# microsoft/UniSpeech

Hardware: AMD Instinct MI355X
Metric: audio-seconds/sec pretraining, WavLM-Base 15s@16kHz (higher is better)
Workload: dtype bf16; 1 GPU; WavLM-Base (12L, d=768) pretrain fwd+bwd+grad-reduce+fused-Adam, bf16, batch=32x15s per GPU, masked-pred loss (BASELINE.json configs[1]); global_batch=32, frames_per_utt=749, parallelism=dp1, optimizer=fused Adam, fp32 master, clip 10

## Files before the change

include/wavlm_hip.h:

```cpp
#ifndef WAVLM_HIP_H
#define WAVLM_HIP_H
#include <stddef.h>
#include <stdint.h>
#ifdef __cplusplus
extern "C" {
#endif

#define WAVLM_HIP_ABI_VERSION 30
int wavlm_abi_version(void);

typedef struct wavlm_gemm_desc {
  int32_t dtype;
  int32_t c_dtype;
  int32_t M, N, K, KB;
  int32_t transA, transB;
  int64_t lda, ldb, ldc;
  int64_t sA_kb, sB_kb;
  int32_t batch_o, batch_i;
  int64_t sA_o, sA_i, sB_o, sB_i, sC_o, sC_i;
  const void* A;
  const void* B;
  void* C;
  float alpha;
  int32_t epi;
// ... 54 lines not shown
                      void* stream);
#define WL_CONV_RELAYOUT_MAX 8
typedef struct {
  const void* W[WL_CONV_RELAYOUT_MAX];
  void* Wf[WL_CONV_RELAYOUT_MAX];
  void* Wb[WL_CONV_RELAYOUT_MAX];
  int32_t Cout[WL_CONV_RELAYOUT_MAX], Cin[WL_CONV_RELAYOUT_MAX], k[WL_CONV_RELAYOUT_MAX], s[WL_CONV_RELAYOUT_MAX];
  int32_t n_layers, dtype;
} wavlm_conv_relayout_desc;
int wavlm_conv_weights_relayout(const wavlm_conv_relayout_desc* d, void* stream);
int wavlm_conv_wgrad_scatter(const wavlm_conv_relayout_desc* d, int32_t accumulate, void* stream);
int wavlm_axpby(const void* x, int32_t x_dtype, void* y, int32_t y_dtype, int64_t n, float a, float b, void* stream);
int wavlm_scale_dev(void* y, int32_t dtype, int64_t n, const float* scalar, float extra, void* stream);
int wavlm_dropout(const void* x, void* y, int64_t n, float p, uint64_t seed, int32_t dtype, void* stream);
int wavlm_dropout_add(const void* x, const void* r, void* y, int64_t n, float p, uint64_t seed, int32_t dtype, void* stream);
int wavlm_replace_mix(const void* x, const void* q, const uint8_t* sel, void* y, int64_t rows, int32_t D, float p, uint64_t seed,
                      int32_t dtype, void* stream);
int wavlm_replace_mix_bwd(const void* g, const uint8_t* sel, void* dx, void* dq, int64_t rows, int32_t D, float p, uint64_t seed,
                          int32_t dtype, void* stream);
uint64_t wavlm_sumsq_workspace_bytes(void);
int wavlm_sumsq(const void* x, int32_t dtype, int64_t n, float scale, float* out, void* workspace, uint64_t ws_bytes,
                void* stream);

uint64_t wavlm_conv0_gn_workspace_bytes(int32_t B, int64_t T, int32_t C, int32_t stride);
int wavlm_conv0_gn_gelu_fwd(const void* wav, int32_t wav_dtype, const void* W, const void* gamma, const void* beta,
                            int32_t param_dtype, void* out, int32_t out_dtype, float* stats, int32_t B, int64_t T,
                            int32_t C, int32_t kw, int32_t stride, float eps, void* workspace, uint64_t ws_bytes,
                            void* stream);
uint64_t wavlm_conv0_gn_bwd_workspace_bytes(int32_t B, int64_t T, int32_t C, int32_t stride);
int wavlm_conv0_gn_gelu_bwd(const void* wav, int32_t wav_dtype, const void* W, const void* gamma, const void* beta,
                            int32_t param_dtype, const void* g, int32_t g_dtype, const float* stats, void* dW,
                            void* dgamma, void* dbeta, int32_t B, int64_t T, int32_t C, int32_t kw, int32_t stride,
                            float gscale, void* workspace, uint64_t ws_bytes, void* stream);

uint64_t wavlm_conv0_ln_fwd_workspace_bytes(void);
int wavlm_conv0_ln_gelu_fwd(const void* wav, int32_t wav_dtype, const void* W, const void* conv_bias, const void* gamma,
                            const void* beta, int32_t param_dtype, void* out, int32_t out_dtype, int32_t B, int64_t T,
                            int32_t C, int32_t kw, int32_t stride, float eps, void* workspace, uint64_t ws_bytes,
                            void* stream);
uint64_t wavlm_conv0_ln_bwd_workspace_bytes(int32_t B, int64_t T, int32_t C, int32_t stride);
int wavlm_conv0_ln_gelu_bwd(const void* wav, int32_t wav_dtype, const void* W, const void* conv_bias, const void* gamma,
                            const void* beta, int32_t param_dtype, const void* g, int32_t g_dtype, void* dW,
                            void* dconv_bias, void* dgamma, void* dbeta, int32_t B, int64_t T, int32_t C, int32_t kw,
                            int32_t stride, float eps, float gscale, void* workspace, uint64_t ws_bytes, void* stream);

int wavlm_relpos_gather(const void* emb, int32_t emb_dtype, const int32_t* bucket, float* tab, int32_t H, int32_t L,
                        void* stream);
int wavlm_relpos_scatter(const float* dtab, const int32_t* bucket, void* demb, int32_t emb_dtype, int32_t H, int32_t L,
                         int32_t num_buckets, void* stream);
int wavlm_gate_fwd(const void* x, const void* W, const void* bias, const void* grep_a, float* gate, float* ga, float* gb,
                   int32_t B, int32_t T, int32_t H, int32_t hd, int32_t dtype, int32_t param_dtype, void* stream);
uint64_t wavlm_gate_bwd_workspace_bytes(int32_t H, int32_t hd);
int wavlm_gate_bwd(const float* dgate, const void* x, const void* W, const void* grep_a, const float* ga,
                   const float* gb, void* dx, void* dW, void* dbias, void* dgrep_a, int32_t B, int32_t T, int32_t H,
                   int32_t hd, int32_t dtype, int32_t param_dtype, int32_t accumulate_params, void* workspace,
                   uint64_t ws_bytes, void* stream);
int wavlm_attn_softmax_fwd(const void* S, void* P, float* lse, const float* gate, const float* tab, const uint8_t* kpm,
                           int32_t B, int32_t H, int32_t T, int64_t ldS, int64_t ldP, int32_t s_dtype, int32_t p_dtype,
                           float p_drop, uint64_t seed, void* stream);
uint64_t wavlm_attn_softmax_bwd_workspace_bytes(int32_t B, int32_t H, int32_t T);
int wavlm_attn_softmax_bwd(const void* S, const void* dP, const float* lse, const float* gate, const float* tab,
                           const uint8_t* kpm, void* dS, float* dgate, float* dtab, int32_t dtab_accumulate, int32_t B,
                           int32_t H, int32_t T, int64_t ldS, int64_t ldP, int32_t s_dtype, int32_t p_dtype,
                           float p_drop, uint64_t seed, void* workspace, uint64_t ws_bytes, void* stream);

int wavlm_attn_fused_fwd(const void* qkv, void* O, float* lse, const float* gate, const float* tab, const uint8_t* kpm,
                         int32_t B, int32_t H, int32_t T, int32_t head_dim, float scale, float p_drop, uint64_t seed,
                         void* stream);
uint64_t wavlm_attn_fused_bwd_workspace_bytes(int32_t B, int32_t H, int32_t T);
int wavlm_attn_fused_bwd(const void* qkv, const void* O, const void* dO, const float* lse, const float* gate,
                         const float* tab, const uint8_t* kpm, void* dqkv, float* dgate, float* dtab, void* dbias,
                         int32_t dbias_dtype, int32_t dbias_accumulate, int32_t B, int32_t H, int32_t T, int32_t head_dim,
                         float scale, float p_drop, uint64_t seed, void* workspace, uint64_t ws_bytes, void* stream);
uint64_t wavlm_attn_fused_pstore_bytes(int32_t B, int32_t H, int32_t T);
uint64_t wavlm_attn_fused_dbits_bytes(int32_t B, int32_t H, int32_t T);
int wavlm_attn_fused_fwd_p(const void* qkv, void* O, float* lse, const float* gate, const float* tab, const uint8_t* kpm,
                           void* pstore, uint64_t pstore_bytes, int32_t B, int32_t H, int32_t T, int32_t head_dim, float scale,
                           float p_drop, uint64_t seed, void* stream);
int wavlm_attn_fused_bwd_p(const void* qkv, const void* O, const void* dO, const float* lse, const float* gate,
                           const float* tab, const uint8_t* kpm, const void* pstore, uint64_t pstore_bytes, void* dqkv,
                           float* dgate, float* dtab, void* dbias, int32_t dbias_dtype, int32_t dbias_accumulate, int32_t B,
                           int32_t H, int32_t T, int32_t head_dim, float scale, float p_drop, uint64_t seed, void* workspace,
                           uint64_t ws_bytes, void* stream);

uint64_t wavlm_posconv_weight_workspace_bytes(int32_t D, int32_t Cg, int32_t K);
int wavlm_posconv_weight_fwd(const void* v, const void* g, int32_t param_dtype, void* Wf, void* Wb, int32_t out_dtype,
                             float* norm, int32_t D, int32_t Cg, int32_t K, int32_t layout, void* workspace,
                             uint64_t ws_bytes, void* stream);
int wavlm_posconv_weight_bwd(const float* dWf, const void* v, const void* g, const float* norm, int32_t param_dtype,
                             void* dv, void* dg, int32_t D, int32_t Cg, int32_t K, int32_t nsplit, void* workspace,
                             uint64_t ws_bytes, void* stream);
int wavlm_posconv_group_major(const void* x, const void* aux, void* out, void* nat_out, int32_t B, int32_t T, int32_t D,
                              int32_t G, int32_t left_pad, int32_t Tp, int32_t dtype, int32_t aux_is_grad, void* stream);

int wavlm_posconv_direct_supported(int32_t Cg, int32_t K, int32_t T);
int wavlm_posconv_direct(const void* xg, const void* W, const void* bias, const void* res, void* out, void* aux,
                         int32_t B, int32_t G, int32_t T, int32_t Tp, int32_t Cg, int32_t K, int32_t gelu, void* stream);
int wavlm_posconv_dw_direct_splits(int32_t Cg, int32_t G);
int wavlm_posconv_dw_direct(const void* xg, const void* dug, float* part, int32_t B, int32_t G, int32_t T, int32_t Tp,
                            int32_t du_off, int32_t Cg, int32_t K, void* stream);

int wavlm_l2norm_fwd(const void* x, int32_t x_dtype, void* y, int32_t y_dtype, float* inv_norm, int64_t rows,
                     int32_t D, float eps, void* stream);
int wavlm_l2norm_bwd(const void* dy, const void* y, int32_t y_dtype, const float* inv_norm, void* dx, int32_t x_dtype,
                     int64_t rows, int32_t D, void* stream);
int wavlm_ce_rows(const float* logits, const int32_t* target, float* loss_rows, float* correct_rows, void* dlogits,
                  int32_t d_dtype, int64_t S, int32_t V, int64_t ld_logits, int64_t ld_dlogits, float weight,
                  int32_t flat_wrong, void* stream);

int wavlm_gather_dot(const void* X, const void* Y, int32_t dtype, const int32_t* idx, float* out, int64_t S, int32_t N,
                     int32_t D, float scale, const void* mask_raw, void* stream);
int wavlm_rows_wsum(const void* Y, int32_t dtype, const int32_t* src, const float* w, const int32_t* off, void* out,
                    int32_t out_dtype, int64_t rows, int32_t D, int32_t accumulate, void* stream);
uint64_t wavlm_bce_workspace_bytes(void);
int wavlm_bce_logits(const float* logits, const uint8_t* targets, float* dlogits, float* out, int64_t n, float gscale,
                     void* workspace, uint64_t ws_bytes, void* stream);
int wavlm_glu_fwd(const void* x, void* y, int64_t rows, int32_t F, int32_t dtype, int32_t gate, void* stream);
int wavlm_glu_bwd(const void* x, const void* dy, void* dx, int64_t rows, int32_t F, int32_t dtype, int32_t gate, void* stream);
int wavlm_act_fwd(const void* x, void* y, int64_t n, int32_t dtype, int32_t kind, void* stream);
int wavlm_act_bwd(const void* x, const void* dy, void* dx, int64_t n, int32_t dtype, int32_t kind, void* stream);
uint64_t wavlm_sum_workspace_bytes(void);
int wavlm_sum_f32(const float* x, int64_t n, float* out, void* workspace, uint64_t ws_bytes, void* stream);

int wavlm_adam_step(float* p, float* m, float* v, const void* grad, int32_t grad_dtype, void* p_lowp,
                    int32_t lowp_dtype, int64_t n, float lr, float beta1, float beta2, float eps, float weight_decay,
                    int64_t step, float grad_mult, const float* grad_mult_dev, const float* gnorm_sq, float max_norm,
                    void* stream);

uint64_t wavlm_mix_workspace_bytes(int32_t B, int64_t T);
int wavlm_mix_utterances(const float* src, float* dst, void* dst_lowp, int32_t B, int64_t T, const int32_t* ops,
                         int32_t n_ops, const int32_t* op_begin, const float* noise, int32_t normalize, float eps,
                         void* workspace, uint64_t ws_bytes, void* stream);

uint64_t wavlm_gumbel_vq_partial_rows(int64_t n);
int wavlm_gumbel_vq_fwd(const void* logits, int32_t dtype, const float* noise, uint64_t seed, float tau, int32_t training,
                        int64_t n, int32_t G, int32_t V, float* ysoft, int32_t* idx, float* part, int64_t ld_part,
                        void* stream);
int wavlm_vq_perplexity(const float* sums, int64_t n, int32_t G, int32_t V, float* out, float* dA, void* stream);
int wavlm_gumbel_vq_bwd(const void* logits, int32_t dtype, const float* ysoft, const float* dret, const float* dA,
                        const float* dppl, float tau, int64_t n, int32_t G, int32_t V, void* dlogits, void* stream);

typedef struct wavlm_layer_desc {
  int32_t B, T, D, H, F;
  int32_t pre_ln;
  int32_t param_dtype;
  int32_t dtab_accumulate;
  float eps1, eps2, scale;
  float p_drop, p_attn;
  int32_t attn_store_p;
  uint64_t seed_r1, seed_r2, seed_attn;
  const void *Wqkv, *bqkv, *Wo, *bo, *W1, *b1, *W2, *b2, *ln1_g, *ln1_b, *ln2_g, *ln2_b;
  const void *Wgate, *bgate, *grep_a;
  void *dWqkv, *dbqkv, *dWo, *dbo, *dW1, *db1, *dW2, *db2, *dln1_g, *dln1_b, *dln2_g, *dln2_b, *dWgate, *dbgate, *dgrep_a;
  void* db2_prev;
  const float* tab;
  const uint8_t* kpm;
  const void* x;
  const void* r_in;
  void* y;
  void* r_out;
  void* saved; uint64_t saved_bytes;
  void* workspace; uint64_t ws_bytes;
  const void* dy;
  const void* dr_out;
  void* dx;
  void* dr_in;
  float* dtab;
} wavlm_layer_desc;
uint64_t wavlm_layer_saved_bytes(const wavlm_layer_desc* d);
uint64_t wavlm_layer_fwd_workspace_bytes(const wavlm_layer_desc* d);
uint64_t wavlm_layer_bwd_workspace_bytes(const wavlm_layer_desc* d);
int wavlm_encoder_layer_fwd(const wavlm_layer_desc* d, void* stream);
int wavlm_encoder_layer_bwd(const wavlm_layer_desc* d, void* stream);

typedef void (*wavlm_grad_listener)(const void* base, uint64_t bytes, void* stream, void* user);
void wavlm_dp_set_listener(wavlm_grad_listener cb, void* user);

int wavlm_dp_unique_id(void* id128);
int wavlm_dp_init(int32_t rank, int32_t world, const void* id128, int32_t average);
int wavlm_dp_bucket_ready(void* base, uint64_t count, int32_t dtype, void* compute_stream);
int wavlm_dp_finish(void* compute_stream);
int wavlm_dp_destroy(void);

uint64_t wavlm_kmeans_centres_bytes(int32_t K, int32_t D);
int wavlm_kmeans_prepare(const float* C, int32_t K, int32_t D, void* image, uint64_t image_bytes, void* stream);
int wavlm_kmeans_assign(const void* X, int32_t x_dtype, int64_t N, int32_t D, int64_t ldx, const void* image, int32_t K,
                        int32_t* labels, float* min_dist, void* stream);
uint64_t wavlm_kmeans_accumulate_workspace_bytes(int64_t N, int32_t K, int32_t D);
int wavlm_kmeans_accumulate(const void* X, int32_t x_dtype, int64_t N, int32_t D, int64_t ldx, const int32_t* labels,
                            int32_t K, float* sums, int32_t* counts, void* workspace, uint64_t ws_bytes, void* stream);
int wavlm_kmeans_update(float* C, float* weights, const float* sums, const int32_t* counts, int32_t K, int32_t D,
                        int32_t mode, void* stream);

int wavlm_spk_mix_norm(const void* const* states, const int64_t* stride_b, const int64_t* stride_t, int32_t n_states,
                       int32_t dtype, const float* weights, const int32_t* lengths, int32_t B, int32_t T, int32_t D,
                       void* out, int32_t out_dtype, int64_t out_stride_b, int64_t out_stride_t, int32_t pad, float add,
                       float eps, void* stream);
int wavlm_spk_rowact(const void* x, int32_t x_dtype, int64_t x_stride_b, int64_t ldx, void* y, int32_t y_dtype,
                     int64_t y_stride_b, int64_t ldy, int32_t B, int32_t T, int32_t C, int32_t act, const float* scale,
                     const float* shift, const int32_t* lengths, float* mean_out, void* stream);
int wavlm_spk_res2(const void* x, int32_t x_dtype, int64_t x_stride_b, int64_t ldx, void* y, int32_t y_dtype,
                   int64_t y_stride_b, int64_t ldy, int32_t B, int32_t T, int32_t C, int32_t dilation, const float* w_image,
                   const float* bias, const float* scale, const float* shift, const int32_t* lengths, void* stream);
uint64_t wavlm_spk_se_workspace_bytes(int32_t B, int32_t C);
int wavlm_spk_se_residual(const void* x, int32_t x_dtype, int64_t x_stride_b, int64_t ldx, const float* mean, const void* w1,
                          const void* b1, const void* w2, const void* b2, int32_t w_dtype, const void* res, int32_t res_dtype,
                          int64_t res_stride_b, int64_t ld_res, void* out, int32_t out_dtype, int64_t out_stride_b,
                          int64_t ld_out, int32_t B, int32_t T, int32_t C, int32_t Cb, const int32_t* lengths,
                          void* workspace, uint64_t ws_bytes, void* stream);
int wavlm_spk_asp(const void* x, int32_t x_dtype, int64_t x_stride_b, int64_t ldx, const void* logits, int32_t l_dtype,
                  int64_t l_stride_b, int64_t ldl, int32_t B, int32_t T, int32_t C, const int32_t* lengths, const float* scale,
                  const float* shift, float* pooled_raw, void* out, int32_t out_dtype, void* stream);

int wavlm_diar_front(const void* const* states, const int64_t* stride_b, const int64_t* stride_t, int32_t n_states,
                     int32_t dtype, const float* weights, int32_t B, int32_t T, int32_t D, int32_t subsampling, int32_t T_out,
                     void* out, int32_t out_dtype, int64_t out_stride_b, int64_t out_stride_t, float add, float eps,
                     void* stream);
int wavlm_attn_plain_fwd(const void* qkv, void* O, int32_t B, int32_t H, int32_t T, int32_t head_dim, int32_t dtype,
                         float scale, void* stream);
int wavlm_diar_estimate(const void* z, int32_t z_dtype, int64_t z_stride_b, int64_t ldz, int32_t B, int32_t T, int32_t S,
                        int32_t E, float* activities, void* vectors, int32_t v_dtype, void* stream);

int wavlm_resample_supported(int32_t o, int32_t n, int32_t width);
int wavlm_resample_rows(const void* x, int32_t x_dtype, int64_t x_stride, int32_t B, int64_t L, const int32_t* lengths,
                        const float* table, const int32_t* first, int32_t o, int32_t n, int32_t width, void* y,
                        int32_t y_dtype, int64_t y_stride, void* stream);

int wavlm_mfcc_supported(int32_t W, int32_t S, int32_t P);
int64_t wavlm_mfcc_frames(int64_t len, int32_t W, int32_t S);
int wavlm_mfcc_rows(const void* x, int32_t x_dtype, int64_t x_stride, int32_t B, int64_t L, const int32_t* lengths, int32_t W,
                    int32_t S, int32_t P, const float* window, const float* twiddle, const int32_t* mel_idx, const float* mel_w,
                    int32_t n_mel_w, const float* dct, float* y, int64_t y_stride, int64_t Mmax, int32_t ncol, void* stream);

int wavlm_fbank_supported(int32_t W, int32_t S, int32_t P, int32_t M);
int64_t wavlm_fbank_frames(int64_t len, int32_t S, int32_t P);
int wavlm_fbank_rows(const void* x, int32_t x_dtype, int64_t x_stride, int32_t B, int64_t L, const int32_t* lengths, int32_t W,
                     int32_t S, int32_t P, int32_t M, const float* window, const float* twiddle, const int32_t* mel_idx,
                     const float* mel_w, int32_t n_mel_w, float* y, int64_t y_stride, int64_t Tmax, void* stream);

int wavlm_ctc_supported(int32_t C, int32_t Lmax);
uint64_t wavlm_ctc_workspace_bytes(int32_t B, int32_t T, int32_t Lmax);
int wavlm_ctc_loss(const void* logits, int32_t dtype, int64_t stride_b, int64_t stride_t, int32_t B, int32_t T, int32_t C,
                   const int32_t* targets, const int32_t* target_offsets, int32_t n_targets, int32_t Lmax,
                   const int32_t* input_lengths, int32_t blank, int32_t zero_infinity, const float* grad_out, float* nll,
                   void* dlogits, void* workspace, uint64_t ws_bytes, void* stream);
int wavlm_ctc_greedy(const void* logits, int32_t dtype, int64_t stride_b, int64_t stride_t, int32_t B, int32_t T, int32_t C,
                     const int32_t* input_lengths, int32_t blank, int32_t* tokens, int32_t* counts, void* stream);

int wavlm_ctc_score_supported(int32_t T, int32_t Lt);
uint64_t wavlm_ctc_score_workspace_bytes(int32_t B, int32_t T, int32_t Lt);
// ... 50 lines not shown
```

unispeech_amd/_lib.py:

```python
import ctypes as C
import os

_HERE = os.path.dirname(os.path.abspath(__file__))
LIB_PATH = os.environ.get("WAVLM_HIP_LIB") or os.path.join(_HERE, "lib", "libwavlm_hip.so")

_lib = None
ABI_VERSION = 30

F32, BF16, I16 = 0, 1, 2

c_i32, c_i64, c_u64, c_f32, c_vp = C.c_int32, C.c_int64, C.c_uint64, C.c_float, C.c_void_p


class ConvRelayoutDesc(C.Structure):
    _fields_ = [("W", c_vp * 8), ("Wf", c_vp * 8), ("Wb", c_vp * 8),
                ("Cout", c_i32 * 8), ("Cin", c_i32 * 8), ("k", c_i32 * 8), ("s", c_i32 * 8),
                ("n_layers", c_i32), ("dtype", c_i32)]


class GemmDesc(C.Structure):
    _fields_ = [
        ("dtype", c_i32), ("c_dtype", c_i32),
        ("M", c_i32), ("N", c_i32), ("K", c_i32), ("KB", c_i32),
        ("transA", c_i32), ("transB", c_i32),
        ("lda", c_i64), ("ldb", c_i64), ("ldc", c_i64),
        ("sA_kb", c_i64), ("sB_kb", c_i64),
        ("batch_o", c_i32), ("batch_i", c_i32),
        ("sA_o", c_i64), ("sA_i", c_i64), ("sB_o", c_i64), ("sB_i", c_i64), ("sC_o", c_i64), ("sC_i", c_i64),
        ("A", c_vp), ("B", c_vp), ("C", c_vp),
        ("alpha", c_f32), ("epi", c_i32),
        ("bias", c_vp), ("bias_dtype", c_i32), ("sBias_o", c_i64), ("sBias_i", c_i64),
        ("aux", c_vp), ("aux_dtype", c_i32), ("ld_aux", c_i64), ("sAux_o", c_i64), ("sAux_i", c_i64),
        ("res", c_vp), ("res_dtype", c_i32), ("ld_res", c_i64), ("sRes_o", c_i64), ("sRes_i", c_i64),
        ("accumulate", c_i32), ("split_k", c_i32),
        ("workspace", c_vp), ("ws_bytes", c_u64),
        ("colsum", c_vp), ("colsum_dtype", c_i32), ("colsum_accumulate", c_i32),
    ]


class WgradItem(C.Structure):
    _fields_ = [("dy", c_vp), ("x", c_vp), ("dW", c_vp), ("N", c_i32), ("K", c_i32)]


class LayerDesc(C.Structure):
    _fields_ = [
        ("B", c_i32), ("T", c_i32), ("D", c_i32), ("H", c_i32), ("F", c_i32),
        ("pre_ln", c_i32), ("param_dtype", c_i32), ("dtab_accumulate", c_i32),
        ("eps1", c_f32), ("eps2", c_f32), ("scale", c_f32), ("p_drop", c_f32), ("p_attn", c_f32),
        ("attn_store_p", c_i32),
        ("seed_r1", c_u64), ("seed_r2", c_u64), ("seed_attn", c_u64),
        ("Wqkv", c_vp), ("bqkv", c_vp), ("Wo", c_vp), ("bo", c_vp), ("W1", c_vp), ("b1", c_vp), ("W2", c_vp), ("b2", c_vp),
        ("ln1_g", c_vp), ("ln1_b", c_vp), ("ln2_g", c_vp), ("ln2_b", c_vp),
        ("Wgate", c_vp), ("bgate", c_vp), ("grep_a", c_vp),
        ("dWqkv", c_vp), ("dbqkv", c_vp), ("dWo", c_vp), ("dbo", c_vp), ("dW1", c_vp), ("db1", c_vp), ("dW2", c_vp),
        ("db2", c_vp), ("dln1_g", c_vp), ("dln1_b", c_vp), ("dln2_g", c_vp), ("dln2_b", c_vp),
        ("dWgate", c_vp), ("dbgate", c_vp), ("dgrep_a", c_vp),
        ("db2_prev", c_vp),
        ("tab", c_vp), ("kpm", c_vp),
        ("x", c_vp), ("r_in", c_vp), ("y", c_vp), ("r_out", c_vp),
        ("saved", c_vp), ("saved_bytes", c_u64), ("workspace", c_vp), ("ws_bytes", c_u64),
        ("dy", c_vp), ("dr_out", c_vp), ("dx", c_vp), ("dr_in", c_vp), ("dtab", c_vp),
    ]


GRAD_LISTENER = C.CFUNCTYPE(None, c_vp, c_u64, c_vp, c_vp)


SIGNATURES = {
    "wavlm_abi_version": (c_i32, []),
    "wavlm_gemm_workspace_bytes": (c_u64, [C.POINTER(GemmDesc)]),
    "wavlm_gemm": (c_i32, [C.POINTER(GemmDesc), c_vp]),
    "wavlm_gemm_grouped": (c_i32, [C.POINTER(GemmDesc), c_i32, c_vp]),
    "wavlm_grid_blocks": (c_i32, []),
    "wavlm_split_single": (c_i32, [c_i32, c_i32, c_i64, c_i32]),
    "wavlm_split_grouped": (c_i32, [c_i64, c_i64, c_i32, c_i32]),
    "wavlm_slabs_grouped": (c_i32, [c_i64, c_i64, c_i32, c_i32, c_i32]),
    "wavlm_wgrad_grouping": (c_i32, []),
    "wavlm_linear_wgrads_workspace_bytes": (c_u64, [C.POINTER(WgradItem), c_i32, c_i64]),
    "wavlm_linear_wgrads": (c_i32, [C.POINTER(WgradItem), c_i32, c_i64, c_i32, c_vp, c_u64, c_vp]),
    "wavlm_layernorm_fwd": (c_i32, [c_vp, c_vp, c_vp, c_vp, c_vp, c_vp, c_vp, c_vp, c_i64, c_i32, c_f32, c_i32, c_i32,
                                    c_i32, c_f32, c_u64, c_f32, c_u64, c_vp]),
    "wavlm_layernorm_bwd_workspace_bytes": (c_u64, [c_i32]),
    "wavlm_layernorm_bwd": (c_i32, [c_vp, c_vp, c_vp, c_vp, c_vp, c_vp, c_vp, c_vp, c_vp, c_vp, c_vp, c_vp, c_i64, c_i32, c_i32,
                                    c_i32, c_i32, c_f32, c_u64, c_f32, c_u64, c_f32, c_i32, c_i32, c_vp, c_u64, c_vp]),
    "wavlm_layernorm_bwd_seg": (c_i32, [c_vp, c_vp, c_vp, c_vp, c_vp, c_vp, c_vp, c_vp, c_vp, c_vp, c_vp, c_vp, c_i64, c_i32, c_i32,
                                        c_i32, c_i32, c_f32, c_u64, c_f32, c_u64, c_f32, c_i32, c_i32, c_i32, c_i32, c_vp, c_u64,
                                        c_vp]),
    "wavlm_colsum_workspace_bytes": (c_u64, [c_i32]),
    "wavlm_colsum": (c_i32, [c_vp, c_i64, c_i32, c_i64, c_i32, c_vp, c_vp, c_vp, c_i32, c_i32, c_vp, c_u64, c_vp]),
    "wavlm_select_rows": (c_i32, [c_vp, c_vp, c_vp, c_vp, c_vp, c_i64, c_i32, c_i32, c_i32, c_vp]),
    "wavlm_gather_rows": (c_i32, [c_vp, c_vp, c_vp, c_i64, c_i32, c_i32, c_vp]),
    "wavlm_conv_weights_relayout": (c_i32, [C.POINTER(ConvRelayoutDesc), c_vp]),
    "wavlm_conv_wgrad_scatter": (c_i32, [C.POINTER(ConvRelayoutDesc), c_i32, c_vp]),
    "wavlm_axpby": (c_i32, [c_vp, c_i32, c_vp, c_i32, c_i64, c_f32, c_f32, c_vp]),
    "wavlm_scale_dev": (c_i32, [c_vp, c_i32, c_i64, c_vp, c_f32, c_vp]),
    "wavlm_dropout": (c_i32, [c_vp, c_vp, c_i64, c_f32, c_u64, c_i32, c_vp]),
    "wavlm_dropout_add": (c_i32, [c_vp, c_vp, c_vp, c_i64, c_f32, c_u64, c_i32, c_vp]),
    "wavlm_replace_mix": (c_i32, [c_vp, c_vp, c_vp, c_vp, c_i64, c_i32, c_f32, c_u64, c_i32, c_vp]),
    "wavlm_replace_mix_bwd": (c_i32, [c_vp, c_vp, c_vp, c_vp, c_i64, c_i32, c_f32, c_u64, c_i32, c_vp]),
    "wavlm_sumsq_workspace_bytes": (c_u64, []),
    "wavlm_sumsq": (c_i32, [c_vp, c_i32, c_i64, c_f32, c_vp, c_vp, c_u64, c_vp]),
    "wavlm_conv0_gn_workspace_bytes": (c_u64, [c_i32, c_i64, c_i32, c_i32]),
    "wavlm_conv0_gn_gelu_fwd": (c_i32, [c_vp, c_i32, c_vp, c_vp, c_vp, c_i32, c_vp, c_i32, c_vp, c_i32, c_i64, c_i32,
                                        c_i32, c_i32, c_f32, c_vp, c_u64, c_vp]),
    "wavlm_conv0_gn_bwd_workspace_bytes": (c_u64, [c_i32, c_i64, c_i32, c_i32]),
    "wavlm_conv0_gn_gelu_bwd": (c_i32, [c_vp, c_i32, c_vp, c_vp, c_vp, c_i32, c_vp, c_i32, c_vp, c_vp, c_vp, c_vp,
                                        c_i32, c_i64, c_i32, c_i32, c_i32, c_f32, c_vp, c_u64, c_vp]),
    "wavlm_conv0_ln_fwd_workspace_bytes": (c_u64, []),
    "wavlm_conv0_ln_gelu_fwd": (c_i32, [c_vp, c_i32, c_vp, c_vp, c_vp, c_vp, c_i32, c_vp, c_i32, c_i32, c_i64, c_i32, c_i32,
                                        c_i32, c_f32, c_vp, c_u64, c_vp]),
    "wavlm_conv0_ln_bwd_workspace_bytes": (c_u64, [c_i32, c_i64, c_i32, c_i32]),
    "wavlm_conv0_ln_gelu_bwd": (c_i32, [c_vp, c_i32, c_vp, c_vp, c_vp, c_vp, c_i32, c_vp, c_i32, c_vp, c_vp, c_vp, c_vp, c_i32,
                                        c_i64, c_i32, c_i32, c_i32, c_f32, c_f32, c_vp, c_u64, c_vp]),
    "wavlm_relpos_gather": (c_i32, [c_vp, c_i32, c_vp, c_vp, c_i32, c_i32, c_vp]),
    "wavlm_relpos_scatter": (c_i32, [c_vp, c_vp, c_vp, c_i32, c_i32, c_i32, c_i32, c_vp]),
    "wavlm_gate_fwd": (c_i32, [c_vp, c_vp, c_vp, c_vp, c_vp, c_vp, c_vp, c_i32, c_i32, c_i32, c_i32, c_i32, c_i32,
                               c_vp]),
    "wavlm_gate_bwd_workspace_bytes": (c_u64, [c_i32, c_i32]),
    "wavlm_gate_bwd": (c_i32, [c_vp, c_vp, c_vp, c_vp, c_vp, c_vp, c_vp, c_vp, c_vp, c_vp, c_i32, c_i32, c_i32, c_i32,
                               c_i32, c_i32, c_i32, c_vp, c_u64, c_vp]),
    "wavlm_attn_softmax_fwd": (c_i32, [c_vp, c_vp, c_vp, c_vp, c_vp, c_vp, c_i32, c_i32, c_i32, c_i64, c_i64, c_i32,
                                       c_i32, c_f32, c_u64, c_vp]),
    "wavlm_attn_softmax_bwd_workspace_bytes": (c_u64, [c_i32, c_i32, c_i32]),
    "wavlm_attn_softmax_bwd": (c_i32, [c_vp, c_vp, c_vp, c_vp, c_vp, c_vp, c_vp, c_vp, c_vp, c_i32, c_i32, c_i32,
                                       c_i32, c_i64, c_i64, c_i32, c_i32, c_f32, c_u64, c_vp, c_u64, c_vp]),
    "wavlm_attn_fused_fwd": (c_i32, [c_vp, c_vp, c_vp, c_vp, c_vp, c_vp, c_i32, c_i32, c_i32, c_i32, c_f32, c_f32, c_u64,
                                     c_vp]),
    "wavlm_attn_fused_bwd_workspace_bytes": (c_u64, [c_i32, c_i32, c_i32]),
    "wavlm_attn_fused_bwd": (c_i32, [c_vp, c_vp, c_vp, c_vp, c_vp, c_vp, c_vp, c_vp, c_vp, c_vp, c_vp, c_i32, c_i32,
                                     c_i32, c_i32, c_i32, c_i32, c_f32, c_f32, c_u64, c_vp, c_u64, c_vp]),
    "wavlm_attn_fused_pstore_bytes": (c_u64, [c_i32, c_i32, c_i32]),
    "wavlm_attn_fused_dbits_bytes": (c_u64, [c_i32, c_i32, c_i32]),
    "wavlm_attn_fused_fwd_p": (c_i32, [c_vp, c_vp, c_vp, c_vp, c_vp, c_vp, c_vp, c_u64, c_i32, c_i32, c_i32, c_i32, c_f32, c_f32,
                                       c_u64, c_vp]),
    "wavlm_attn_fused_bwd_p": (c_i32, [c_vp, c_vp, c_vp, c_vp, c_vp, c_vp, c_vp, c_vp, c_u64, c_vp, c_vp, c_vp, c_vp, c_i32, c_i32,
                                       c_i32, c_i32, c_i32, c_i32, c_f32, c_f32, c_u64, c_vp, c_u64, c_vp]),
    "wavlm_posconv_weight_workspace_bytes": (c_u64, [c_i32, c_i32, c_i32]),
    "wavlm_posconv_weight_fwd": (c_i32, [c_vp, c_vp, c_i32, c_vp, c_vp, c_i32, c_vp, c_i32, c_i32, c_i32, c_i32, c_vp,
                                         c_u64, c_vp]),
    "wavlm_posconv_dw_direct_splits": (c_i32, [c_i32, c_i32]),
    "wavlm_posconv_dw_direct": (c_i32, [c_vp, c_vp, c_vp, c_i32, c_i32, c_i32, c_i32, c_i32, c_i32, c_i32, c_vp]),
    "wavlm_posconv_weight_bwd": (c_i32, [c_vp, c_vp, c_vp, c_vp, c_i32, c_vp, c_vp, c_i32, c_i32, c_i32, c_i32, c_vp, c_u64,
                                         c_vp]),
    "wavlm_posconv_direct_supported": (c_i32, [c_i32, c_i32, c_i32]),
    "wavlm_posconv_direct": (c_i32, [c_vp, c_vp, c_vp, c_vp, c_vp, c_vp, c_i32, c_i32, c_i32, c_i32, c_i32, c_i32, c_i32,
                                     c_vp]),
    "wavlm_posconv_group_major": (c_i32, [c_vp, c_vp, c_vp, c_vp, c_i32, c_i32, c_i32, c_i32, c_i32, c_i32, c_i32,
                                          c_i32, c_vp]),
    "wavlm_l2norm_fwd": (c_i32, [c_vp, c_i32, c_vp, c_i32, c_vp, c_i64, c_i32, c_f32, c_vp]),
    "wavlm_l2norm_bwd": (c_i32, [c_vp, c_vp, c_i32, c_vp, c_vp, c_i32, c_i64, c_i32, c_vp]),
    "wavlm_ce_rows": (c_i32, [c_vp, c_vp, c_vp, c_vp, c_vp, c_i32, c_i64, c_i32, c_i64, c_i64, c_f32, c_i32, c_vp]),
    "wavlm_gather_dot": (c_i32, [c_vp, c_vp, c_i32, c_vp, c_vp, c_i64, c_i32, c_i32, c_f32, c_vp, c_vp]),
    "wavlm_rows_wsum": (c_i32, [c_vp, c_i32, c_vp, c_vp, c_vp, c_vp, c_i32, c_i64, c_i32, c_i32, c_vp]),
    "wavlm_bce_workspace_bytes": (c_u64, []),
    "wavlm_bce_logits": (c_i32, [c_vp, c_vp, c_vp, c_vp, c_i64, c_f32, c_vp, c_u64, c_vp]),
    "wavlm_glu_fwd": (c_i32, [c_vp, c_vp, c_i64, c_i32, c_i32, c_i32, c_vp]),
    "wavlm_glu_bwd": (c_i32, [c_vp, c_vp, c_vp, c_i64, c_i32, c_i32, c_i32, c_vp]),
    "wavlm_act_fwd": (c_i32, [c_vp, c_vp, c_i64, c_i32, c_i32, c_vp]),
    "wavlm_act_bwd": (c_i32, [c_vp, c_vp, c_vp, c_i64, c_i32, c_i32, c_vp]),
    "wavlm_sum_workspace_bytes": (c_u64, []),
    "wavlm_sum_f32": (c_i32, [c_vp, c_i64, c_vp, c_vp, c_u64, c_vp]),
    "wavlm_adam_step": (c_i32, [c_vp, c_vp, c_vp, c_vp, c_i32, c_vp, c_i32, c_i64, c_f32, c_f32, c_f32, c_f32, c_f32,
                                c_i64, c_f32, c_vp, c_vp, c_f32, c_vp]),
    "wavlm_mix_workspace_bytes": (c_u64, [c_i32, c_i64]),
    "wavlm_mix_utterances": (c_i32, [c_vp, c_vp, c_vp, c_i32, c_i64, c_vp, c_i32, c_vp, c_vp, c_i32, c_f32, c_vp, c_u64, c_vp]),
    "wavlm_gumbel_vq_partial_rows": (c_u64, [c_i64]),
    "wavlm_gumbel_vq_fwd": (c_i32, [c_vp, c_i32, c_vp, c_u64, c_f32, c_i32, c_i64, c_i32, c_i32, c_vp, c_vp, c_vp, c_i64, c_vp]),
    "wavlm_vq_perplexity": (c_i32, [c_vp, c_i64, c_i32, c_i32, c_vp, c_vp, c_vp]),
    "wavlm_gumbel_vq_bwd": (c_i32, [c_vp, c_i32, c_vp, c_vp, c_vp, c_vp, c_f32, c_i64, c_i32, c_i32, c_vp, c_vp]),
    "wavlm_layer_saved_bytes": (c_u64, [C.POINTER(LayerDesc)]),
    "wavlm_layer_fwd_workspace_bytes": (c_u64, [C.POINTER(LayerDesc)]),
    "wavlm_layer_bwd_workspace_bytes": (c_u64, [C.POINTER(LayerDesc)]),
    "wavlm_encoder_layer_fwd": (c_i32, [C.POINTER(LayerDesc), c_vp]),
    "wavlm_encoder_layer_bwd": (c_i32, [C.POINTER(LayerDesc), c_vp]),
    "wavlm_kmeans_centres_bytes": (c_u64, [c_i32, c_i32]),
    "wavlm_kmeans_prepare": (c_i32, [c_vp, c_i32, c_i32, c_vp, c_u64, c_vp]),
    "wavlm_kmeans_assign": (c_i32, [c_vp, c_i32, c_i64, c_i32, c_i64, c_vp, c_i32, c_vp, c_vp, c_vp]),
    "wavlm_kmeans_accumulate_workspace_bytes": (c_u64, [c_i64, c_i32, c_i32]),
    "wavlm_kmeans_accumulate": (c_i32, [c_vp, c_i32, c_i64, c_i32, c_i64, c_vp, c_i32, c_vp, c_vp, c_vp, c_u64, c_vp]),
    "wavlm_kmeans_update": (c_i32, [c_vp, c_vp, c_vp, c_vp, c_i32, c_i32, c_i32, c_vp]),
    "wavlm_spk_mix_norm": (c_i32, [c_vp, c_vp, c_vp, c_i32, c_i32, c_vp, c_vp, c_i32, c_i32, c_i32, c_vp, c_i32, c_i64, c_i64,
                                   c_i32, c_f32, c_f32, c_vp]),
    "wavlm_spk_rowact": (c_i32, [c_vp, c_i32, c_i64, c_i64, c_vp, c_i32, c_i64, c_i64, c_i32, c_i32, c_i32, c_i32, c_vp, c_vp,
                                 c_vp, c_vp, c_vp]),
    "wavlm_spk_res2": (c_i32, [c_vp, c_i32, c_i64, c_i64, c_vp, c_i32, c_i64, c_i64, c_i32, c_i32, c_i32, c_i32, c_vp, c_vp,
                               c_vp, c_vp, c_vp, c_vp]),
    "wavlm_spk_se_workspace_bytes": (c_u64, [c_i32, c_i32]),
    "wavlm_spk_se_residual": (c_i32, [c_vp, c_i32, c_i64, c_i64, c_vp, c_vp, c_vp, c_vp, c_vp, c_i32, c_vp, c_i32, c_i64, c_i64,
                                      c_vp, c_i32, c_i64, c_i64, c_i32, c_i32, c_i32, c_i32, c_vp, c_vp, c_u64, c_vp]),
    "wavlm_spk_asp": (c_i32, [c_vp, c_i32, c_i64, c_i64, c_vp, c_i32, c_i64, c_i64, c_i32, c_i32, c_i32, c_vp, c_vp, c_vp, c_vp,
                              c_vp, c_i32, c_vp]),
    "wavlm_diar_front": (c_i32, [c_vp, c_vp, c_vp, c_i32, c_i32, c_vp, c_i32, c_i32, c_i32, c_i32, c_i32, c_vp, c_i32, c_i64, c_i64,
                                 c_f32, c_f32, c_vp]),
    "wavlm_attn_plain_fwd": (c_i32, [c_vp, c_vp, c_i32, c_i32, c_i32, c_i32, c_i32, c_f32, c_vp]),
    "wavlm_diar_estimate": (c_i32, [c_vp, c_i32, c_i64, c_i64, c_i32, c_i32, c_i32, c_i32, c_vp, c_vp, c_i32, c_vp]),
    "wavlm_resample_supported": (c_i32, [c_i32, c_i32, c_i32]),
    "wavlm_resample_rows": (c_i32, [c_vp, c_i32, c_i64, c_i32, c_i64, c_vp, c_vp, c_vp, c_i32, c_i32, c_i32, c_vp, c_i32, c_i64,
                                    c_vp]),
    "wavlm_mfcc_supported": (c_i32, [c_i32, c_i32, c_i32]),
    "wavlm_mfcc_frames": (c_i64, [c_i64, c_i32, c_i32]),
    "wavlm_mfcc_rows": (c_i32, [c_vp, c_i32, c_i64, c_i32, c_i64, c_vp, c_i32, c_i32, c_i32, c_vp, c_vp, c_vp, c_vp, c_i32, c_vp,
                                c_vp, c_i64, c_i64, c_i32, c_vp]),
    "wavlm_fbank_supported": (c_i32, [c_i32, c_i32, c_i32, c_i32]),
    "wavlm_fbank_frames": (c_i64, [c_i64, c_i32, c_i32]),
    "wavlm_fbank_rows": (c_i32, [c_vp, c_i32, c_i64, c_i32, c_i64, c_vp, c_i32, c_i32, c_i32, c_i32, c_vp, c_vp, c_vp, c_vp, c_i32,
                                 c_vp, c_i64, c_i64, c_vp]),
    "wavlm_ctc_supported": (c_i32, [c_i32, c_i32]),
    "wavlm_ctc_workspace_bytes": (c_u64, [c_i32, c_i32, c_i32]),
    "wavlm_ctc_loss": (c_i32, [c_vp, c_i32, c_i64, c_i64, c_i32, c_i32, c_i32, c_vp, c_vp, c_i32, c_i32, c_vp, c_i32, c_i32, c_vp,
                               c_vp, c_vp, c_vp, c_u64, c_vp]),
    "wavlm_ctc_greedy": (c_i32, [c_vp, c_i32, c_i64, c_i64, c_i32, c_i32, c_i32, c_vp, c_i32, c_vp, c_vp, c_vp]),
    "wavlm_ctc_score_supported": (c_i32, [c_i32, c_i32]),
    "wavlm_ctc_score_workspace_bytes": (c_u64, [c_i32, c_i32, c_i32]),
    "wavlm_ctc_score": (c_i32, [c_vp, c_i32, c_i64, c_i64, c_i32, c_i32, c_i32, c_vp, c_i32, c_vp, c_i32, c_i32, c_i32, c_vp, c_i32,
                                c_vp, c_vp, c_vp, c_vp, c_u64, c_vp]),
    "wavlm_ctc_beam_supported": (c_i32, [c_i32, c_i32, c_i32, c_i32]),
    "wavlm_ctc_beam_workspace_bytes": (c_u64, [c_i32, c_i32, c_i32]),
    "wavlm_ctc_beam": (c_i32, [c_vp, c_i32, c_i64, c_i64, c_i32, c_i32, c_i32, c_vp, c_i32, c_i32, c_i32, c_vp, c_vp, c_vp, c_vp,
                               c_vp, c_vp, c_vp, c_i32, c_i32, c_i32, c_i32, c_i32, c_i32, c_i32, c_f32, c_f32, c_f32, c_i32, c_vp,
# ... 53 lines not shown
```

unispeech_amd/csrc/attn_fused.hip:

```cpp
#include "attn_fused.hpp"

typedef float f32x2_t __attribute__((ext_vector_type(2)));
#if !defined(WAVLM_EXPERIMENTAL)
#undef FA_FWD_LAZY
#undef FA_FWD_THETA
#undef FA_DQ_PK
#endif
#ifndef FA_FWD_LAZY
#define FA_FWD_LAZY 0
#endif
#ifndef FA_FWD_THETA
#define FA_FWD_THETA 8.f
#endif
#ifndef FA_DQ_PK
#define FA_DQ_PK 1
#endif
#if !defined(WAVLM_EXPERIMENTAL)
#undef FA_FWD_MFMA_SUM
#endif
#ifndef FA_FWD_MFMA_SUM
#define FA_FWD_MFMA_SUM 0
#endif
#ifndef FA_FWD_BIAS_IN_C
#define FA_FWD_BIAS_IN_C 1
// ... 405 lines not shown
    for (int j = threadIdx.x; j < p.Tkb; j += 256)
      kb[j] = (j < T && !(p.kpm && p.kpm[(long)b * T + j])) ? 0.f : -INFINITY;
    if constexpr (DROP && !BCONS)
      for (int jp = threadIdx.x; jp < (p.Tkb >> 1); jp += 256) colw[jp] = fa_col_word(p.s1, (unsigned)jp);
  }
  for (int q = threadIdx.x; q < SKEW_BYTES / 16; q += 256) reinterpret_cast<uint4*>(smem + 32768)[q] = make_uint4(0, 0, 0, 0);
  const float g = p.gate ? p.gate[(long)bh * T + ic] : 0.f;
  const float g2 = g * FA_LOG2E;
  const float nlse2 = valid_i ? p.log2sc - p.lse[(long)bh * T + ic] * FA_LOG2E : -INFINITY;
#if FA_DQ_BIAS_IN_C
  const float g2s = g2 / p.sc2, nlse2s = nlse2 / p.sc2;
#endif
  const unsigned roww = fa_row_word(p.s0, (unsigned)(bh * T + ic));
  const float* trow = tabs + (T - 1 - ic);
  unsigned short* sk_w = reinterpret_cast<unsigned short*>(skew + (31 - ql + 4 * hi) * 64 + 2 * ql);
  const unsigned char* sk_r = skew + (lane & 15) * 64 + (lane >> 4) * 16;
  const unsigned sk_w3 = (unsigned)(unsigned long)(las_ptr)(skew + ql * FA_SKEW_RB + 2 * (31 - ql + 4 * hi));
  const unsigned char* sk_r3 = skew + (8 * (lane >> 4) + ((lane & 15) >> 2)) * FA_SKEW_RB + 8 * (lane & 3);
  const unsigned ktr = fa_tr_base(lane);

  f32x16_t dq[2];
#pragma unroll
  for (int f = 0; f < 2; ++f)
#pragma unroll
    for (int r = 0; r < 16; ++r) dq[f][r] = 0.f;
  f32x4_t dacc[6];
#pragma unroll
  for (int c = 0; c < 6; ++c) dacc[c] = f32x4_t{0.f, 0.f, 0.f, 0.f};
  U4 gfrag; gfrag.v = make_uint4(0, 0, 0, 0);
  if constexpr (TAB) {
    unsigned short* gb = gball + wave_u * 32;
    if (hi == 0) gb[ql] = f2bf(g);
    __builtin_amdgcn_s_waitcnt(0xc07f);
    __builtin_amdgcn_wave_barrier();
    gfrag.v = *reinterpret_cast<const uint4*>(gb + (lane >> 4) * 8);
  }
  float dg = 0.f;
#if FA_DQ_PK
  f32x2_t dg2 = f32x2_t{0.f, 0.f};
#endif
  const int nkv = (T + FA_BKV - 1) / FA_BKV;
  unsigned bacc0 = 0, bacc1 = 0, pend_bits = 0;
  int pend_bits_jt = -1;
  unsigned* dbp = nullptr;
  const unsigned thsv = (unsigned)p.ths;
  if constexpr (EMIT)
    if (p.dbits) dbp = p.dbits + ((long)bh * p.db_nkb + hi) * p.db_Tq + fa_bitrow(i);
  const unsigned* bsrc = nullptr;
  unsigned nxt0 = 0, nxt1 = 0;
  if constexpr (BCONS) {
    bsrc = p.dbits + (long)bh * p.db_nkb * p.db_Tq + fa_bitrow(i);
    nxt0 = bsrc[0]; nxt1 = bsrc[p.db_Tq];
  }

  const unsigned char* pld = nullptr;
  const float* mtp = nullptr;
  U4 pA0[2], pA1[2], pB0[2], pB1[2];
  float mtA = 0.f, mtB = 0.f;
  auto p_load = [&](int jn, U4 (&x0)[2], U4 (&x1)[2], float& mx) __attribute__((always_inline)) {
    const unsigned char* src = pld + (long)jn * FA_PTILE_BYTES;
#pragma unroll
    for (int s2 = 0; s2 < 2; ++s2) {
      x0[s2].v = *reinterpret_cast<const uint4*>(src + s2 * 1024);
      x1[s2].v = *reinterpret_cast<const uint4*>(src + (2 + s2) * 1024);
    }
    mx = mtp[(long)jn * p.ps.Tq];
  };
  if constexpr (SP) {
    pld = p.ps.P16 + (((long)bh * p.ps.nq32 + (qblk * 4 + wave_u)) * p.ps.nkv) * FA_PTILE_BYTES + lane * 16;
    mtp = p.ps.mt + (long)bh * p.ps.nkv * p.ps.Tq + (qblk * FA_BQ + 32 * wave_u + ql);
    p_load(0, pA0, pA1, mtA);
    p_load(p.ps.nkv > 1 ? 1 : 0, pB0, pB1, mtB);
  }
#if FA_TILE_SRC
  FaTileSrc ksrc, vsrc;
  ksrc.init(base + D, D3, T);
  vsrc.init(base + 2 * D, D3, T);
#endif
  FA_LOAD_KV(0, kbuf(0), vbuf(0));
  fa_tile_sync();

  float pend_v = 0.f;
  int pend_d = -1;
  auto skew_sums = [&](int j0p) __attribute__((always_inline)) {
    f32x4_t nacc[6];
#pragma unroll
    for (int cb = 0; cb < 6; ++cb) {
      U4 bfr;
#if FA_DQ_SKEW_ROWS
      {
        const bf16x4_t lo = __builtin_amdgcn_ds_read_tr16_b64_v4bf16((lds_b4_ptr)(sk_r3 + cb * 32));
        const bf16x4_t hi4 = __builtin_amdgcn_ds_read_tr16_b64_v4bf16((lds_b4_ptr)(sk_r3 + 4 * FA_SKEW_RB + cb * 32));
        bfr.b = __builtin_shufflevector(lo, hi4, 0, 1, 2, 3, 4, 5, 6, 7);
      }
#else
      bfr.v = *reinterpret_cast<const uint4*>(sk_r + cb * 1024);
#endif
      const f32x4_t cin = cb < 2 ? dacc[cb + 4] : f32x4_t{0.f, 0.f, 0.f, 0.f};
      nacc[cb] = __builtin_amdgcn_mfma_f32_16x16x32_bf16(gfrag.b, bfr.b, cin, 0, 0, 0);
    }
#pragma unroll
    for (int cb = 0; cb < 6; ++cb) dacc[cb] = nacc[cb];
    const int gsel = lane >> 4;
    const float a0 = dacc[0][0], a1 = dacc[1][0], a2 = dacc[2][0], a3 = dacc[3][0];
    float v = a0;
    v = gsel == 1 ? a1 : v;
    v = gsel == 2 ? a2 : v;
    v = gsel == 3 ? a3 : v;
    pend_v = v;
    pend_d = dlo0 + j0p + lane;
  };
  auto flush_pending = [&]() __attribute__((always_inline)) {
    if (pend_d >= 0 && pend_d < L) prow[pend_d] = pend_v;
    pend_d = -1;
  };
  int cur = 0;
  auto tile_body = [&](int jt, U4 (&x0)[2], U4 (&x1)[2], float& mx) __attribute__((always_inline)) {
    const int j0 = jt * FA_BKV;
    const bool more = jt + 1 < nkv;
    U4 pc0[2], pc1[2];
    float ct = 0.f;
    if constexpr (SP) {
#pragma unroll
      for (int s2 = 0; s2 < 2; ++s2)
#pragma unroll
        for (int e = 0; e < 4; ++e) {
          asm volatile("v_mov_b32 %0, %1" : "=v"(pc0[s2].u[e]) : "v"(x0[s2].u[e]));
          asm volatile("v_mov_b32 %0, %1" : "=v"(pc1[s2].u[e]) : "v"(x1[s2].u[e]));
        }
      ct = mx > -INFINITY ? __builtin_amdgcn_exp2f(mx + nlse2) : 0.f;
    }
    if (more) {
      FA_LOAD_KV(j0 + FA_BKV, kbuf(cur ^ 1), vbuf(cur ^ 1));
    }
    if constexpr (SP && !(FA_SP_PROBE & 1)) p_load(jt + 2 < nkv ? jt + 2 : jt, x0, x1, mx);
    if constexpr (TAB) flush_pending();
    unsigned bw0 = 0, bw1 = 0;
    if constexpr (BCONS) {
      bw0 = nxt0 >> (8 * (1 - hi)); bw1 = nxt1 >> (8 * (1 - hi));
      const int jn = more ? jt + 1 : jt;
      nxt0 = bsrc[(long)jn * 2 * p.db_Tq]; nxt1 = bsrc[((long)jn * 2 + 1) * p.db_Tq];
    }
    if constexpr (EMIT) {
      if (dbp && pend_bits_jt >= 0) dbp[(long)pend_bits_jt * 2 * p.db_Tq] = pend_bits;
      pend_bits_jt = -1;
    }
    if constexpr (TAB && FA_DQ_DEFER) {
      if (jt > 0) skew_sums(j0 - FA_BKV);
    }
    constexpr bool PF = FA_DQ_PREFETCH && TAB;
    float tvv[PF ? 2 : 1][16];
    unsigned cww[PF ? 2 : 1][8];
    if constexpr (PF) {
#pragma unroll
      for (int f = 0; f < 2; ++f)
#pragma unroll
        for (int r = 0; r < 16; ++r) {
          const int j = j0 + 32 * f + (r & 3) + 8 * (r >> 2) + 4 * hi;
          tvv[f][r] = trow[j];
          if (DROP && !SP && !BCONS && !(r & 1)) cww[f][r >> 1] = (colw + ((j0 + 4 * hi) >> 1))[(32 * f + (r & 3) + 8 * (r >> 2)) >> 1];
        }
    }
    const bool edge = !SP && ((p.kpm != nullptr) || (j0 + FA_BKV > T));
    U4 dsf0[2], dsf1[2];
    f32x16_t s[2], dp[2];
    using F0 = std::integral_constant<int, 0>;
    using F1 = std::integral_constant<int, 1>;
    auto scores = [&](auto fc) __attribute__((always_inline)) {
      constexpr int f = decltype(fc)::value;
#if FA_DQ_BIAS_IN_C
#pragma unroll
      for (int r = 0; r < 16; ++r) {
        const int j = j0 + 32 * f + (r & 3) + 8 * (r >> 2) + 4 * hi;
        float tv;
        if constexpr (PF) tv = tvv[f][r]; else tv = trow[j];
        float c = fmaf(g2s, tv, nlse2s);
        if (edge) c += kb[j];
        s[f][r] = c; dp[f][r] = 0.f;
      }
#else
#pragma unroll
      for (int r = 0; r < 16; ++r) { s[f][r] = 0.f; dp[f][r] = 0.f; }
#endif
#pragma unroll
      for (int kk = 0; kk < 4; ++kk) {
        if constexpr (!SP)
          s[f] = __builtin_amdgcn_mfma_f32_32x32x16_bf16(frag_plain(kbuf(cur), 32 * f + ql, kk, hi), qf[kk].b, s[f], 0, 0, 0);
        dp[f] = __builtin_amdgcn_mfma_f32_32x32x16_bf16(frag_plain(vbuf(cur), 32 * f + ql, kk, hi), dof[kk].b, dp[f], 0, 0, 0);
      }
    };
    auto elem_pass = [&](auto fc, auto edge_c) __attribute__((always_inline)) {
      constexpr int f = decltype(fc)::value;
      constexpr bool EDGE = decltype(edge_c)::value;
#pragma unroll
      for (int r = 0; r < 16; r += 2) {
        float dv[2];
        unsigned w = 0;
        if constexpr (DROP && !SP && !BCONS) {
          if constexpr (PF) w = fa_mix(roww + cww[f][r >> 1]);
          else w = fa_mix(roww + (colw + ((j0 + 4 * hi) >> 1))[(32 * f + (r & 3) + 8 * (r >> 2)) >> 1]);
        }
        if constexpr (SP) {
          const f16x2_t h2 = __builtin_bit_cast(f16x2_t, (f == 0 ? pc0 : pc1)[r >> 3].u[(r & 7) >> 1]);
          const f32x2_t ps2 = f32x2_t{(float)h2[0], (float)h2[1]} * f32x2_t{ct, ct};
          const f32x2_t pk2 = f32x2_t{fmaxf(ps2[0], 0.f), fmaxf(ps2[1], 0.f)};
          const f32x2_t pa2 = f32x2_t{__builtin_fabsf(ps2[0]), __builtin_fabsf(ps2[1])};
          const f32x2_t ds2 = __builtin_elementwise_fma(pk2, f32x2_t{dp[f][r], dp[f][r + 1]}, -(pa2 * f32x2_t{dls, dls}));
          dv[0] = ds2[0]; dv[1] = ds2[1];
          if constexpr (TAB) {
            f32x2_t tv2;
            if constexpr (PF) tv2 = f32x2_t{tvv[f][r], tvv[f][r + 1]};
            else { const int j = j0 + 32 * f + (r & 3) + 8 * (r >> 2) + 4 * hi; tv2 = f32x2_t{trow[j], trow[j + 1]}; }
#if FA_DQ_PK
            dg2 = __builtin_elementwise_fma(ds2, tv2, dg2);
#else
            dg = fmaf(ds2[0], tv2[0], fmaf(ds2[1], tv2[1], dg));
#endif
          }
        } else
// ... 61 lines not shown
#endif
          const float pe = __builtin_amdgcn_exp2f(x);
          float dpe = dp[f][rr];
          if constexpr (DROP) dpe = (e ? fa_keep_hi(w, p.ths) : fa_keep_lo(w, p.ths)) ? dpe : 0.f;
          const float ds = pe * (dpe - dls);
          dv[e] = ds;
          dg = fmaf(ds, tv, dg);
        }
#endif
        const unsigned u2 = pack_bf16(dv[0], dv[1]);
        if constexpr (f == 0) dsf0[r >> 3].u[(r & 7) >> 1] = u2; else dsf1[r >> 3].u[(r & 7) >> 1] = u2;
        if constexpr (TAB) {
          const int dd = 32 * f + (r & 3) + 8 * (r >> 2);
#if !FA_DQ_NOSKEW && !(FA_SP_PROBE & 4)
#if FA_DQ_SKEW_ROWS
          if (r & 2) {
            const unsigned prev = (f == 0 ? dsf0 : dsf1)[r >> 3].u[((r & 7) >> 1) - 1];
            const unsigned long pair = ((unsigned long)u2 << 32) | prev;
            const unsigned a = sk_w3 + 2 * (dd - 2);
            asm volatile("ds_write_b64 %0, %1" :: "v"(a), "v"(pair) : "memory");
          }
#else
          sk_w[dd * 32] = (unsigned short)u2;
          sk_w[(dd + 1) * 32] = (unsigned short)(u2 >> 16);
#endif
#endif
        }
      }
    };
    auto dq_acc = [&](auto fc) __attribute__((always_inline)) {
      constexpr int f = decltype(fc)::value;
#pragma unroll
      for (int f2 = 0; f2 < 2; ++f2)
#pragma unroll
        for (int s2 = 0; s2 < 2; ++s2)
          dq[f2] = __builtin_amdgcn_mfma_f32_32x32x16_bf16(frag_tr(kbuf(cur), ktr, f2, f, s2), (f == 0 ? dsf0[s2] : dsf1[s2]).b, dq[f2], 0, 0, 0);
    };
#if FA_DQ_BOTH
    scores(F0{}); scores(F1{});
    if (edge) { elem_pass(F0{}, std::true_type{}); elem_pass(F1{}, std::true_type{}); }
    else { elem_pass(F0{}, std::false_type{}); elem_pass(F1{}, std::false_type{}); }
    dq_acc(F0{}); dq_acc(F1{});
#else
    scores(F0{});
    if (edge) elem_pass(F0{}, std::true_type{}); else elem_pass(F0{}, std::false_type{});
    dq_acc(F0{});
    scores(F1{});
    if (edge) elem_pass(F1{}, std::true_type{}); else elem_pass(F1{}, std::false_type{});
    dq_acc(F1{});
#endif
    if constexpr (EMIT) {
      auto spread = [&](unsigned a) __attribute__((always_inline)) {
        unsigned x = __builtin_bitreverse32(a) >> 16;
        x = (x | (x << 8)) & 0x00FF00FFu;
        x = (x | (x << 4)) & 0x0F0F0F0Fu;
        return x << (4 * hi);
      };
      unsigned w0 = spread(bacc0), w1 = spread(bacc1);
      asm volatile("s_nop 1\n\tv_permlane32_swap_b32 %0, %1\n\ts_nop 1" : "+v"(w0), "+v"(w1));
      pend_bits = w0 | w1;
      pend_bits_jt = jt;
      bacc0 = 0; bacc1 = 0;
    }
    if constexpr (TAB && !FA_DQ_DEFER) skew_sums(j0);
    fa_tile_sync<SP ? 5 : 0>();
    cur ^= 1;
  };
  if constexpr (SP) {
    for (int pi = 0; pi < (nkv >> 1); ++pi) {
      tile_body(2 * pi, pA0, pA1, mtA);
      tile_body(2 * pi + 1, pB0, pB1, mtB);
    }
    if (nkv & 1) tile_body(nkv - 1, pA0, pA1, mtA);
  } else {
    for (int jt = 0; jt < nkv; ++jt) tile_body(jt, pA0, pA1, mtA);
  }
  if constexpr (TAB && FA_DQ_DEFER) skew_sums((nkv - 1) * FA_BKV);
  if constexpr (TAB) flush_pending();
  if constexpr (EMIT)
    if (dbp && pend_bits_jt >= 0) dbp[(long)pend_bits_jt * 2 * p.db_Tq] = pend_bits;
  if (TAB && lane < 32) {
    const float v = lane < 16 ? dacc[4][0] : dacc[5][0];
    const int d = dlo0 + 64 * nkv + lane;
    if (d >= 0 && d < L) prow[d] = v;
  }
#if FA_DQ_PK
  dg = dg2[0] + dg2[1];
#endif
  dg = wl_sum_xor32(dg);
  if (p.dbias_part)
    fa_wave_colsum(dq, p.scale, reinterpret_cast<float*>(smem),
                   p.dbias_part + (((long)b * p.nqb + qblk) * 4 + wave_u) * D3 + h * FA_HD, lane, wave_u);
  if (valid_i) {
    bf16_t* dst = p.dqkv + ((long)b * T + i) * D3 + h * FA_HD;
#pragma unroll
    for (int f2 = 0; f2 < 2; ++f2)
#pragma unroll
      for (int q4 = 0; q4 < 4; ++q4) {
        uint2 w;
        w.x = pack_bf16(dq[f2][4 * q4] * p.scale, dq[f2][4 * q4 + 1] * p.scale);
        w.y = pack_bf16(dq[f2][4 * q4 + 2] * p.scale, dq[f2][4 * q4 + 3] * p.scale);
        *reinterpret_cast<uint2*>(dst + 32 * f2 + 8 * q4 + 4 * hi) = w;
      }
    if (hi == 0) {
      p.delta[(long)bh * T + i] = dl;
      if (p.dgate) p.dgate[(long)bh * T + i] = dg;
    }
  }
}

__global__ __launch_bounds__(1024) void fa_dtab_reduce_kernel(const float* __restrict__ part, float* __restrict__ out,
                                                              int B, int H, int nqt, int L, int Lp, int T, int nkv, int accumulate) {
  __shared__ float4 red[64][17];
  const int col = threadIdx.x & 15, slice = threadIdx.x >> 4;
  const int d = (blockIdx.x * 16 + col) * 4;
  const int h = blockIdx.y;
  const int nrow = nqt * 4, ntot = B * nrow, span = 64 * nkv + 32;
  float4 acc[4];
#pragma unroll
  for (int u = 0; u < 4; ++u) acc[u] = make_float4(0.f, 0.f, 0.f, 0.f);
  if (d < Lp) {
    for (int r0 = slice; r0 < ntot; r0 += 256) {
#pragma unroll
      for (int u = 0; u < 4; ++u) {
        const int r = r0 + 64 * u;
        if (r < ntot) {
          const int b = r / nrow, c = r - b * nrow;
          const int k0 = d - (T - 1 - 32 * c - 31);
          if (k0 > -4 && k0 < span) {
            const float4 v = *reinterpret_cast<const float4*>(part + (((long)b * H + h) * nrow + c) * Lp + d);
            acc[u].x += (k0 >= 0 && k0 < span) ? v.x : 0.f;
            acc[u].y += (k0 + 1 >= 0 && k0 + 1 < span) ? v.y : 0.f;
            acc[u].z += (k0 + 2 >= 0 && k0 + 2 < span) ? v.z : 0.f;
            acc[u].w += (k0 + 3 >= 0 && k0 + 3 < span) ? v.w : 0.f;
          }
        }
      }
    }
  }
  float4 t;
  t.x = (acc[0].x + acc[1].x) + (acc[2].x + acc[3].x); t.y = (acc[0].y + acc[1].y) + (acc[2].y + acc[3].y);
  t.z = (acc[0].z + acc[1].z) + (acc[2].z + acc[3].z); t.w = (acc[0].w + acc[1].w) + (acc[2].w + acc[3].w);
  red[slice][col] = t;
  __syncthreads();
  if (slice < 4) {
    float4 q = make_float4(0.f, 0.f, 0.f, 0.f);
#pragma unroll
    for (int k = 0; k < 16; ++k) { const float4 v = red[slice * 16 + k][col]; q.x += v.x; q.y += v.y; q.z += v.z; q.w += v.w; }
    red[slice * 16][col] = q;
  }
  __syncthreads();
  if (slice == 0 && d < L) {
    const float4 a0 = red[0][col], a1 = red[16][col], a2 = red[32][col], a3 = red[48][col];
    const float o[4] = {(a0.x + a1.x) + (a2.x + a3.x), (a0.y + a1.y) + (a2.y + a3.y), (a0.z + a1.z) + (a2.z + a3.z),
                        (a0.w + a1.w) + (a2.w + a3.w)};
#pragma unroll
    for (int k = 0; k < 4; ++k)
      if (d + k < L) out[(long)h * L + d + k] = accumulate ? out[(long)h * L + d + k] + o[k] : o[k];
  }
}

static FaP fa_params(int B, int H, int T, float scale, float p_drop, uint64_t seed) {
  FaP p;
  p.B = B; p.H = H; p.T = T; p.scale = scale;
  p.sc2 = scale * FA_LOG2E;
  double tt = (double)p_drop * 65536.0 + 0.5; if (tt > 65535.0) tt = 65535.0;
  p.th = p_drop > 0.f ? (unsigned)tt : 0u;
  if (p_drop > 0.f && p.th == 0u) p.th = 1u;
  p.sc = p.th ? (float)(1.0 / (1.0 - (double)p.th / 65536.0)) : 1.f;
  p.log2sc = log2f(p.sc); p.inv_sc = 1.f / p.sc;
  p.ths = (int)p.th - 32768;
  p.k2 = (unsigned)((p.ths - 1) & 0xffff) * 0x10001u;
  p.k3 = (unsigned)(p.ths & 0xffff) * 0x10001u;
  p.ps.P16 = nullptr; p.ps.mt = nullptr;
  p.dbits = nullptr; p.db_fwd = 0; p.db_nkb = ((T + FA_BKV - 1) / FA_BKV) * 2; p.db_Tq = ((T + FA_BQ - 1) / FA_BQ) * FA_BQ;
  p.ps.nq32 = ((T + FA_BQ - 1) / FA_BQ) * 4; p.ps.nkv = (T + FA_BKV - 1) / FA_BKV; p.ps.Tq = ((T + FA_BQ - 1) / FA_BQ) * FA_BQ;
  p.s0 = (unsigned)seed; p.s1 = (unsigned)(seed >> 32);
  const int nkv = (T + FA_BKV - 1) / FA_BKV;
  p.Tkb = nkv * FA_BKV;
  p.Ltab = (T + p.Tkb + 3) & ~3;
  p.qkv = nullptr; p.O = nullptr; p.lse = nullptr; p.gate = nullptr; p.tab = nullptr; p.kpm = nullptr;
  p.dO = nullptr; p.dqkv = nullptr; p.delta = nullptr; p.dgate = nullptr; p.dtab_part = nullptr; p.dbias_part = nullptr;
  return p;
}

extern "C" {

uint64_t wavlm_attn_fused_pstore_bytes(int32_t B, int32_t H, int32_t T) {
  if (B <= 0 || H <= 0 || T <= 0) return 0;
  if (T > FA_PSTORE_MAX_T) return 0;
  return ((fa_pstore_p_bytes(B, H, T) + 255) & ~(uint64_t)255) + fa_pstore_mt_bytes(B, H, T);
}

uint64_t wavlm_attn_fused_dbits_bytes(int32_t B, int32_t H, int32_t T) {
  if (B <= 0 || H <= 0 || T <= 0) return 0;
  return fa_dbits_bytes(B, H, T);
}

int wavlm_attn_fused_fwd(const void* qkv, void* O, float* lse, const float* gate, const float* tab, const uint8_t* kpm,
                         int32_t B, int32_t H, int32_t T, int32_t head_dim, float scale, float p_drop, uint64_t seed,
                         void* stream) {
  return wavlm_attn_fused_fwd_p(qkv, O, lse, gate, tab, kpm, nullptr, 0, B, H, T, head_dim, scale, p_drop, seed, stream);
}

static void fa_bind_pstore(FaP& p, void* pstore, int B, int H, int T) {
  p.ps.P16 = (unsigned char*)pstore;
  p.ps.mt = (float*)((unsigned char*)pstore + ((fa_pstore_p_bytes(B, H, T) + 255) & ~(uint64_t)255));
}

int wavlm_attn_fused_fwd_p(const void* qkv, void* O, float* lse, const float* gate, const float* tab, const uint8_t* kpm,
                           void* pstore, uint64_t pstore_bytes, int32_t B, int32_t H, int32_t T, int32_t head_dim, float scale,
                           float p_drop, uint64_t seed, void* stream) {
  if (!qkv || !O || !lse || B <= 0 || H <= 0 || T <= 0 || head_dim != FA_HD) return WL_EINVAL;
  if ((gate == nullptr) != (tab == nullptr)) return WL_EINVAL;
  const bool bitmode = pstore && pstore_bytes == fa_dbits_bytes(B, H, T);
  if (bitmode) { if ((uintptr_t)pstore & 255) return WL_EINVAL; }
  else if (pstore && (T > FA_PSTORE_MAX_T || pstore_bytes < wavlm_attn_fused_pstore_bytes(B, H, T) || ((uintptr_t)pstore & 15))) return WL_EINVAL;
  FaP p = fa_params(B, H, T, scale, p_drop, seed);
  p.qkv = (const bf16_t*)qkv; p.O = (bf16_t*)O; p.lse = lse; p.gate = gate; p.tab = tab; p.kpm = kpm;
  if (bitmode) { p.dbits = (unsigned*)pstore; p.db_fwd = 1; pstore = nullptr; }
  if (pstore) fa_bind_pstore(p, pstore, B, H, T);
  const size_t smem = 32768 + (size_t)(p.Ltab + p.Tkb + p.Tkb / 2) * sizeof(float);
  p.nqb = (T + FA_BQ - 1) / FA_BQ;
  const dim3 grid((unsigned)(p.nqb * B * H));
  WlProfScope prof(WL_PROF_ATTN_FWD, WL_BF16, 4.0 * B * H * (double)T * T * FA_HD,
                   (double)B * T * H * FA_HD * 2.0 * 4.0 + (double)B * H * T * 4.0, (hipStream_t)stream);
#define FA_FWD(DR, ST) do { if (fa_set_smem(attn_fwd_kernel<DR, ST>, smem) != WL_OK) return WL_ELAUNCH; \
    WL_LAUNCH((attn_fwd_kernel<DR, ST>), grid, dim3(256), smem, (hipStream_t)stream, p); } while (0)
  if (p.th && p.dbits) {
    if (fa_set_smem(attn_fwd_kernel<true, false, true>, smem) != WL_OK) return WL_ELAUNCH;
    WL_LAUNCH((attn_fwd_kernel<true, false, true>), grid, dim3(256), smem, (hipStream_t)stream, p);
  } else
  if (p.th) { if (pstore) FA_FWD(true, true); else FA_FWD(true, false); }
  else { if (pstore) FA_FWD(false, true); else FA_FWD(false, false); }
#undef FA_FWD
  return wl_check_launch();
}

uint64_t wavlm_attn_fused_bwd_workspace_bytes(int32_t B, int32_t H, int32_t T) {
  const uint64_t nqt = (uint64_t)((T + FA_BQ - 1) / FA_BQ);
  const uint64_t Lp = (2 * (uint64_t)T - 1 + 3) & ~(uint64_t)3;
  const uint64_t f = ((uint64_t)B * H * nqt * 4 * Lp + (uint64_t)B * H * T + (uint64_t)B * nqt * 4 * 3 * H * FA_HD) * sizeof(float);
  return ((f + 255) & ~(uint64_t)255) + fa_dbits_bytes(B, H, T);
}

int wavlm_attn_fused_bwd(const void* qkv, const void* O, const void* dO, const float* lse, const float* gate,
                         const float* tab, const uint8_t* kpm, void* dqkv, float* dgate, float* dtab, void* dbias,
                         int32_t dbias_dtype, int32_t dbias_accumulate, int32_t B, int32_t H, int32_t T, int32_t head_dim,
                         float scale, float p_drop, uint64_t seed, void* workspace, uint64_t ws_bytes, void* stream) {
  return wl_attn_fused_bwd_ex(qkv, O, dO, lse, gate, tab, kpm, nullptr, 0, dqkv, dgate, dtab, 0, dbias, dbias_dtype, dbias_accumulate,
                              B, H, T, head_dim, scale, p_drop, seed, workspace, ws_bytes, stream);
}

int wavlm_attn_fused_bwd_p(const void* qkv, const void* O, const void* dO, const float* lse, const float* gate,
                           const float* tab, const uint8_t* kpm, const void* pstore, uint64_t pstore_bytes, void* dqkv,
                           float* dgate, float* dtab, void* dbias, int32_t dbias_dtype, int32_t dbias_accumulate, int32_t B,
                           int32_t H, int32_t T, int32_t head_dim, float scale, float p_drop, uint64_t seed, void* workspace,
                           uint64_t ws_bytes, void* stream) {
  if (pstore && pstore_bytes == fa_dbits_bytes(B, H, T)) { if ((uintptr_t)pstore & 255) return WL_EINVAL; }
  else if (pstore && (T > FA_PSTORE_MAX_T || pstore_bytes < wavlm_attn_fused_pstore_bytes(B, H, T) || ((uintptr_t)pstore & 15))) return WL_EINVAL;
  return wl_attn_fused_bwd_ex(qkv, O, dO, lse, gate, tab, kpm, pstore, pstore_bytes, dqkv, dgate, dtab, 0, dbias, dbias_dtype, dbias_accumulate,
                              B, H, T, head_dim, scale, p_drop, seed, workspace, ws_bytes, stream);
}

}

int wl_attn_fused_bwd_ex(const void* qkv, const void* O, const void* dO, const float* lse, const float* gate,
                         const float* tab, const uint8_t* kpm, const void* pstore, uint64_t pstore_bytes, void* dqkv, float* dgate,
                         float* dtab, int dtab_accumulate,
                         void* dbias, int32_t dbias_dtype, int32_t dbias_accumulate, int32_t B, int32_t H, int32_t T,
                         int32_t head_dim, float scale, float p_drop, uint64_t seed, void* workspace, uint64_t ws_bytes,
                         void* stream) {
  if (!qkv || !O || !dO || !lse || !dqkv || !workspace || B <= 0 || H <= 0 || T <= 0 || head_dim != FA_HD)
    return WL_EINVAL;
  if ((gate == nullptr) != (tab == nullptr)) return WL_EINVAL;
  if (tab && (!dgate || !dtab)) return WL_EINVAL;
  if (ws_bytes < wavlm_attn_fused_bwd_workspace_bytes(B, H, T)) return WL_EINVAL;
  hipStream_t st = (hipStream_t)stream;
  FaP p = fa_params(B, H, T, scale, p_drop, seed);
  p.qkv = (const bf16_t*)qkv; p.O = (bf16_t*)const_cast<void*>(O); p.lse = const_cast<float*>(lse);
  p.gate = gate; p.tab = tab; p.kpm = kpm; p.dO = (const bf16_t*)dO; p.dqkv = (bf16_t*)dqkv; p.dgate = dgate;
  const unsigned* fwd_bits = nullptr;
  if (pstore && pstore_bytes == fa_dbits_bytes(B, H, T)) { fwd_bits = (const unsigned*)pstore; pstore = nullptr; }
  if (pstore) fa_bind_pstore(p, const_cast<void*>(pstore), B, H, T);
  const int nqt = (T + FA_BQ - 1) / FA_BQ;
  const int L = 2 * T - 1;
  p.dtab_part = (float*)workspace;
  const int Lp = (L + 3) & ~3;
  p.delta = p.dtab_part + (long)B * H * nqt * 4 * Lp;
  if (dbias) p.dbias_part = p.delta + (long)B * H * T;
  static const bool dbits_on = []() { const char* e = getenv("WAVLM_ATTN_DBITS"); return e && e[0] == '1'; }();
  static const bool dkv64_on = []() { const char* e = getenv("WAVLM_ATTN_DKV64"); return e && e[0] == '1'; }();
  bool use64 = dkv64_on && dbits_on && !pstore;
  if (use64) {
    FaP q = p; q.nqb = (T + FA_K64 - 1) / FA_K64;
    if (fa_dkv64_smem(q) > 160 * 1024) use64 = false;
  }
  if (fwd_bits && p.th) {
    p.dbits = const_cast<unsigned*>(fwd_bits); p.db_fwd = 1; use64 = false;
  } else
  if (dbits_on && !pstore && p.th) {
    const uint64_t fbytes = ((uint64_t)B * H * nqt * 4 * Lp + (uint64_t)B * H * T + (uint64_t)B * nqt * 4 * 3 * H * FA_HD) * sizeof(float);
    p.dbits = (unsigned*)((unsigned char*)workspace + ((fbytes + 255) & ~(uint64_t)255));
  }
  size_t smem1 = 32768 + (tab ? 4 * FA_SKEW_WAVE : 0) + (size_t)(p.Ltab + p.Tkb + p.Tkb / 2) * sizeof(float) + 256;
  if (smem1 < FA_CS_FLOATS * sizeof(float)) smem1 = FA_CS_FLOATS * sizeof(float);
  p.nqb = nqt;
  WlProfScope prof(WL_PROF_ATTN_BWD, WL_BF16, 10.0 * B * H * (double)T * T * FA_HD,
                   (double)B * T * H * FA_HD * 2.0 * 8.0 + (double)B * H * T * 8.0, st);
#define FA_DQ(DR, TB, SP_) do { if (fa_set_smem(attn_bwd_dq_kernel<DR, TB, SP_>, smem1) != WL_OK) return WL_ELAUNCH; \
    WL_LAUNCH((attn_bwd_dq_kernel<DR, TB, SP_>), dim3((unsigned)(nqt * B * H)), dim3(256), smem1, st, p); } while (0)
#define FA_DQB(TB) do { if (fa_set_smem(attn_bwd_dq_kernel<true, TB, false, true>, smem1) != WL_OK) return WL_ELAUNCH; \
    WL_LAUNCH((attn_bwd_dq_kernel<true, TB, false, true>), dim3((unsigned)(nqt * B * H)), dim3(256), smem1, st, p); } while (0)
  if (p.th && p.db_fwd) {
    if (tab) FA_DQB(true); else FA_DQB(false);
  } else
  if (pstore) {
    if (tab) FA_DQ(false, true, true); else FA_DQ(false, false, true);
  } else if (p.th && p.dbits) {
    if (tab) { if (fa_set_smem(attn_bwd_dq_kernel<true, true, false, false, true>, smem1) != WL_OK) return WL_ELAUNCH;
               WL_LAUNCH((attn_bwd_dq_kernel<true, true, false, false, true>), dim3((unsigned)(nqt * B * H)), dim3(256), smem1, st, p); }
    else { if (fa_set_smem(attn_bwd_dq_kernel<true, false, false, false, true>, smem1) != WL_OK) return WL_ELAUNCH;
           WL_LAUNCH((attn_bwd_dq_kernel<true, false, false, false, true>), dim3((unsigned)(nqt * B * H)), dim3(256), smem1, st, p); }
  } else if (p.th) {
    if (tab) FA_DQ(true, true, false); else FA_DQ(true, false, false);
  } else {
    if (tab) FA_DQ(false, true, false); else FA_DQ(false, false, false);
  }
#undef FA_DQ
#undef FA_DQB
  size_t smem2 = 32768 + (size_t)(p.Ltab + 64) * sizeof(float) + 2 * 4096;
  if (smem2 < FA_CS_FLOATS * sizeof(float)) smem2 = FA_CS_FLOATS * sizeof(float);
  if (use64) {
    p.nqb = (T + FA_K64 - 1) / FA_K64;
    const int rc = fa_launch_dkv64(p, (unsigned)(p.nqb * B * H), st);
    if (rc != WL_OK) return rc;
  } else {
    p.nqb = (T + FA_BK1 - 1) / FA_BK1;
    const dim3 grid2((unsigned)(p.nqb * B * H));
    const int rc = fa_launch_dkv(p, grid2.x, smem2, st);
    if (rc != WL_OK) return rc;
  }
  if (dbias) {
    const int rcb = wl_colsum_finish(p.dbias_part, B * nqt * 4, 3 * H * FA_HD, dbias, dbias_dtype, dbias_accumulate, st);
    if (rcb != WL_OK) return rcb;
    if (dbias_accumulate && !wl_fin_active()) wl_notify_grad(dbias, (uint64_t)3 * H * FA_HD * wl_esize(dbias_dtype), stream);
  }
  if (tab)
    WL_LAUNCH(fa_dtab_reduce_kernel, dim3((unsigned)((Lp / 4 + 15) / 16), (unsigned)H), dim3(1024), 0, st,
              (const float*)p.dtab_part, dtab, (int)B, (int)H, nqt, L, Lp, (int)T, (T + FA_BKV - 1) / FA_BKV, (int)dtab_accumulate);
  return wl_check_launch();
}
```

unispeech_amd/csrc/attn_fused.hpp:

```cpp
#pragma once
#include "tile_loaders.hpp"
#include "../../include/wavlm_hip.h"

typedef __attribute__((ext_vector_type(4))) float f32x4_t;
typedef __attribute__((ext_vector_type(4))) __bf16 bf16x4_t;
typedef __attribute__((address_space(3))) bf16x4_t* lds_b4_ptr;

#define FA_HD 64
#define FA_BQ 128
#define FA_BKV 64
#define FA_BK1 128
#define FA_BQ1 64
#define FA_K64 256

__device__ __forceinline__ unsigned fa_row_word(unsigned s0, unsigned grow) { return hash32(grow ^ s0); }
__device__ __forceinline__ unsigned fa_col_word(unsigned s1, unsigned jpair) { return hash32((jpair ^ s1) + 0x68E31DA4u); }
__device__ __forceinline__ unsigned fa_mix(unsigned x) { return drop_mix(x); }
typedef short s16x2_t __attribute__((ext_vector_type(2)));
__device__ __forceinline__ unsigned fa_dropmask2(unsigned w, unsigned k3) {
  s16x2_t d = __builtin_elementwise_sub_sat(__builtin_bit_cast(s16x2_t, w), __builtin_bit_cast(s16x2_t, k3));
  d = d >> (short)15;
  return __builtin_bit_cast(unsigned, d);
}
__device__ __forceinline__ unsigned fa_keepmask2(unsigned w, unsigned k2) {
// ... 23 lines not shown
__device__ __forceinline__ unsigned fa_tr_base(int lane) {
  const int hi = lane >> 5, li = lane & 15, g1 = (lane >> 4) & 1;
  return (unsigned)((4 * hi + (li >> 2)) * 128 + ((((g1 ^ hi) << 1) | (((li >> 1) & 1) ^ (li >> 3))) << 4) + (li & 1) * 8);
}
__device__ __forceinline__ bf16x8_t frag_tr(const unsigned char* tile, unsigned tr_base, int f2, int f, int s) {
  const unsigned char* kt = tile + tr_base + (32 * f + 16 * s) * 128;
  const bf16x4_t lo = __builtin_amdgcn_ds_read_tr16_b64_v4bf16((lds_b4_ptr)(kt + (f2 << 6)));
  const bf16x4_t hi4 = __builtin_amdgcn_ds_read_tr16_b64_v4bf16((lds_b4_ptr)(kt + 8 * 128 + ((f2 ^ 1) << 6)));
  return __builtin_shufflevector(lo, hi4, 0, 1, 2, 3, 4, 5, 6, 7);
}

#ifndef FA_ASM_DMA
#define FA_ASM_DMA 1
#endif
#if !defined(WAVLM_EXPERIMENTAL)
#undef FA_SP_PROBE
#endif
#ifndef FA_SP_PROBE
#define FA_SP_PROBE 0
#endif
__device__ __forceinline__ void fa_dma16(const void* lane_ptr, unsigned char* ldst) {
#if FA_ASM_DMA
  const unsigned lds_dst = (unsigned)(unsigned long)(las_ptr)ldst;
  asm volatile("s_mov_b32 m0, %0\n\ts_nop 0\n\tglobal_load_lds_dwordx4 %1, off" :: "s"(lds_dst), "v"(lane_ptr) : "memory", "m0");
#else
  __builtin_amdgcn_global_load_lds((gas_ptr)lane_ptr, (las_ptr)ldst, 16, 0, 0);
#endif
}
template <int N = 0> __device__ __forceinline__ void fa_tile_sync() {
#if FA_ASM_DMA && !(FA_SP_PROBE & 16)
  static_assert(N >= 0 && N < 64, "vmcnt is a 6-bit counter");
  __builtin_amdgcn_s_waitcnt(0x0f70 | (N & 15) | ((N >> 4) << 14));
#endif
  __syncthreads();
}

__device__ __forceinline__ void glds_tile64(const bf16_t* base, long ld, int row0, int nrows, unsigned char* lds,
                                            int wave_u) {
  const int t = threadIdx.x;
#pragma unroll
  for (int ps = 0; ps < 2; ++ps) {
    const int rr = (t >> 3) + 32 * ps;
    int row = row0 + rr; if (row > nrows - 1) row = nrows - 1;
    const bf16_t* src = base + (long)row * ld + (((t & 7) ^ ((rr >> 1) & 7)) << 3);
    fa_dma16(src, lds + (ps * 32 + wave_u * 8) * 128);
  }
}

__device__ __forceinline__ void fa_block_map(int nqb, int BH, int& qb, int& bh) {
  const int L = blockIdx.x;
  if ((BH & 7) == 0) {
    const int xcd = L & 7, idx = L >> 3;
    bh = (idx / nqb) * 8 + xcd;
    qb = idx - (idx / nqb) * nqb;
  } else {
    bh = L / nqb;
    qb = L - bh * nqb;
  }
}

#define FA_PTILE_BYTES 4096
#define FA_PSTORE_MAX_T 1024
struct FaPstore { unsigned char* P16; float* mt; int nq32, nkv, Tq; };
__host__ __device__ inline uint64_t fa_pstore_p_bytes(int B, int H, int T) {
  const uint64_t nq32 = (uint64_t)((T + FA_BQ - 1) / FA_BQ) * 4, nkv = (uint64_t)((T + FA_BKV - 1) / FA_BKV);
  return (uint64_t)B * H * nq32 * nkv * FA_PTILE_BYTES;
}
__host__ __device__ inline uint64_t fa_pstore_mt_bytes(int B, int H, int T) {
  const uint64_t Tq = (uint64_t)((T + FA_BQ - 1) / FA_BQ) * FA_BQ, nkv = (uint64_t)((T + FA_BKV - 1) / FA_BKV);
  return (uint64_t)B * H * nkv * Tq * sizeof(float);
}

struct FaP {
  const bf16_t* qkv; bf16_t* O; float* lse;
  const float* gate; const float* tab; const unsigned char* kpm;
  const bf16_t* dO; bf16_t* dqkv; float* delta; float* dgate; float* dtab_part;
  float* dbias_part;
  int B, H, T; float scale; float sc2; unsigned th; float sc, log2sc, inv_sc; unsigned s0, s1;
  int ths; unsigned k2;
  unsigned k3;
  FaPstore ps;
  unsigned* dbits; int db_nkb, db_Tq;
  int db_fwd;
  int Ltab, Tkb;
  int nqb;
};


#define FA_CS_LD 68
#define FA_CS_FLOATS (4 * 32 * FA_CS_LD)
__device__ __forceinline__ void fa_wave_colsum(const f32x16_t (&a)[2], float scale, float* red, float* dst, int lane,
                                               int wave) {
  const int hi = lane >> 5, ql = lane & 31;
  float* buf = red + wave * (32 * FA_CS_LD);
#pragma unroll
  for (int f2 = 0; f2 < 2; ++f2)
#pragma unroll
    for (int q4 = 0; q4 < 4; ++q4) {
      const float4 v = make_float4(a[f2][4 * q4] * scale, a[f2][4 * q4 + 1] * scale, a[f2][4 * q4 + 2] * scale,
                                   a[f2][4 * q4 + 3] * scale);
      *reinterpret_cast<float4*>(buf + ql * FA_CS_LD + 32 * f2 + 8 * q4 + 4 * hi) = v;
    }
  asm volatile("" ::: "memory");
  float s0 = 0.f, s1 = 0.f, s2 = 0.f, s3 = 0.f;
#pragma unroll
  for (int r = 0; r < 32; r += 4) {
    s0 += buf[r * FA_CS_LD + lane]; s1 += buf[(r + 1) * FA_CS_LD + lane];
    s2 += buf[(r + 2) * FA_CS_LD + lane]; s3 += buf[(r + 3) * FA_CS_LD + lane];
  }
  dst[lane] = (s0 + s1) + (s2 + s3);
  asm volatile("" ::: "memory");
}

#ifndef FA_TILE_SRC
#define FA_TILE_SRC 0
#endif
struct FaTileSrc {
  const bf16_t* lane_ptr[2];
  const bf16_t* base; long ld; int nrows;
  __device__ __forceinline__ void init(const bf16_t* base_, long ld_, int nrows_) {
    base = base_; ld = ld_; nrows = nrows_;
    const int t = threadIdx.x;
#pragma unroll
    for (int ps = 0; ps < 2; ++ps) {
      const int rr = (t >> 3) + 32 * ps;
      lane_ptr[ps] = base_ + (long)rr * ld_ + (((t & 7) ^ ((rr >> 1) & 7)) << 3);
    }
  }
  __device__ __forceinline__ void issue(int row0, unsigned char* lds, int wave_u) const {
    if (row0 + 64 <= nrows) {
      const long off = (long)row0 * ld;
#pragma unroll
      for (int ps = 0; ps < 2; ++ps) fa_dma16(lane_ptr[ps] + off, lds + (ps * 32 + wave_u * 8) * 128);
    } else {
      glds_tile64(base, ld, row0, nrows, lds, wave_u);
    }
  }
};

__host__ __device__ inline int fa_bitrow(int i) { return (i & ~7) + 2 * (i & 3) + ((i >> 2) & 1); }
__host__ __device__ inline int fa_fbit_of_key(int k) {
  const int hi = (k >> 2) & 1, r = (k & 3) + 4 * (k >> 3);
  return (r >> 1) + 16 * (r & 1) + 8 * (1 - hi);
}
__host__ __device__ inline uint64_t fa_dbits_bytes(int B, int H, int T) {
  const uint64_t nkb = (uint64_t)((T + FA_BKV - 1) / FA_BKV) * 2, Tq = (uint64_t)((T + FA_BQ - 1) / FA_BQ) * FA_BQ;
  return (uint64_t)B * H * nkb * Tq * sizeof(unsigned) + 256;
}
typedef unsigned u32x8_t __attribute__((ext_vector_type(8)));
typedef const __attribute__((address_space(4))) u32x8_t* fa_mask_ptr;
typedef fa_mask_ptr k64_mask_ptr;
__device__ __forceinline__ float k64_keep(float v, unsigned lo, unsigned hi) {
  const unsigned long m = ((unsigned long)hi << 32) | lo;
  float r;
  asm("s_nop 0\n\tv_cndmask_b32_e64 %0, 0, %1, %2" : "=v"(r) : "v"(v), "s"(m));
  return r;
}
int fa_launch_dkv64(const FaP& p, unsigned grid, hipStream_t st);
size_t fa_dkv64_smem(const FaP& p);

int fa_launch_dkv(const FaP& p, unsigned grid, size_t smem, hipStream_t st);

template <typename K> static int fa_set_smem(K kernel, size_t bytes) {
  if (bytes <= 65536) return WL_OK;
  return hipFuncSetAttribute((const void*)kernel, hipFuncAttributeMaxDynamicSharedMemorySize, (int)bytes) == hipSuccess
             ? WL_OK : WL_ELAUNCH;
// ... 2 lines not shown
```

unispeech_amd/csrc/common.hpp:

```cpp
#pragma once
#include <hip/hip_runtime.h>
#include <stdint.h>
#include <stdio.h>
#include <mutex>

#define WL_MAX_DEVICES 64

#define WL_OK 0
#define WL_EINVAL (-1)
#define WL_ELAUNCH (-2)
#define WL_ENOMEM (-3)

enum { WL_F32 = 0, WL_BF16 = 1, WL_I16 = 2 };

typedef unsigned short bf16_t;

__device__ __forceinline__ float bf2f(bf16_t v) {
  return __uint_as_float(((unsigned)v) << 16);
}
__device__ __forceinline__ bf16_t f2bf(float f) {
  const __bf16 h = (__bf16)f;
  return __builtin_bit_cast(bf16_t, h);
}
__device__ __forceinline__ unsigned pack_bf16x2(float a, float b) {
// ... 82 lines not shown
  return fmaf(x * 0.39894228040143267794f, e, cdf);
}
__device__ __forceinline__ float gelu_both_f(float x, float& grad) {
  float e;
  const float cdf = 0.5f * (1.0f + erf_as(x * 0.70710678118654752440f, e));
  grad = fmaf(x * 0.39894228040143267794f, e, cdf);
  return x * cdf;
}

__device__ __forceinline__ unsigned hash32(unsigned x) {
  x *= 0x9E3779B1u;
  x ^= x >> 15; x *= 0x85EBCA77u;
  x ^= x >> 13; x *= 0xC2B2AE3Du;
  x ^= x >> 16;
  return x;
}
__device__ __forceinline__ unsigned drop_mix(unsigned x) {
  x ^= x >> 16;
  unsigned r;
  asm("v_mul_u32_u24 %0, 0xb5297b, %1" : "=v"(r) : "v"(x));
  return r;
}
static inline unsigned drop_thresh16(float p) {
  if (p <= 0.f) return 0u;
  double t = (double)p * 65536.0 + 0.5;
  if (t > 65535.0) t = 65535.0;
  return t < 1.0 ? 1u : (unsigned)t;
}
static inline float drop_scale16(unsigned th16) { return th16 ? (float)(1.0 / (1.0 - (double)th16 / 65536.0)) : 1.f; }

struct Philox4 { unsigned x, y, z, w; };
__device__ __forceinline__ Philox4 philox4x32_10(unsigned long long seed, unsigned long long ctr) {
  unsigned k0 = (unsigned)seed, k1 = (unsigned)(seed >> 32);
  unsigned c0 = (unsigned)ctr, c1 = (unsigned)(ctr >> 32), c2 = 0x243F6A88u, c3 = 0x85A308D3u;
#pragma unroll
  for (int r = 0; r < 10; ++r) {
    const unsigned long long p0 = (unsigned long long)0xD2511F53u * c0;
    const unsigned long long p1 = (unsigned long long)0xCD9E8D57u * c2;
    const unsigned n0 = (unsigned)(p1 >> 32) ^ c1 ^ k0;
    const unsigned n1 = (unsigned)p1;
    const unsigned n2 = (unsigned)(p0 >> 32) ^ c3 ^ k1;
    const unsigned n3 = (unsigned)p0;
    c0 = n0; c1 = n1; c2 = n2; c3 = n3;
    k0 += 0x9E3779B9u; k1 += 0xBB67AE85u;
  }
  Philox4 o; o.x = c0; o.y = c1; o.z = c2; o.w = c3; return o;
}
__device__ __forceinline__ bool dropout_keep(unsigned long long seed, unsigned long long idx, unsigned thresh) {
  const Philox4 r = philox4x32_10(seed, idx >> 2);
  const unsigned sel = (unsigned)(idx & 3);
  const unsigned v = sel == 0 ? r.x : sel == 1 ? r.y : sel == 2 ? r.z : r.w;
  return v >= thresh;
}

static thread_local int wl_launch_failed = 0;
#define WL_LAUNCH(...)                                            \
  do {                                                            \
    (void)hipGetLastError();                                      \
    hipLaunchKernelGGL(__VA_ARGS__);                              \
    const hipError_t wl_e_ = hipGetLastError();                   \
    if (wl_e_ != hipSuccess) {                                    \
      wl_launch_failed = 1;                                       \
      fprintf(stderr, "[wavlm_hip] kernel launch failed: %s (%s:%d)\n", hipGetErrorString(wl_e_), __FILE__, __LINE__); \
    }                                                             \
  } while (0)
int wl_prof_begin(int cls, int dtype, double flops, double bytes, hipStream_t st);
void wl_prof_end(int i, hipStream_t st);
struct WlProfScope {
  int i; hipStream_t st;
  WlProfScope(int cls, int dtype, double flops, double bytes, hipStream_t s) : i(wl_prof_begin(cls, dtype, flops, bytes, s)), st(s) {}
  ~WlProfScope() { wl_prof_end(i, st); }
};

static inline int wl_check_launch() {
  const int e = wl_launch_failed;
  wl_launch_failed = 0;
  return e ? WL_ELAUNCH : WL_OK;
}

void wl_notify_grad(const void* base, uint64_t bytes, void* stream);
static inline uint64_t wl_esize(int dt) { return dt == WL_BF16 ? 2 : 4; }
int wl_attn_fused_bwd_ex(const void* qkv, const void* O, const void* dO, const float* lse, const float* gate,
                         const float* tab, const uint8_t* kpm, const void* pstore, uint64_t pstore_bytes, void* dqkv, float* dgate,
                         float* dtab, int dtab_accumulate,
                         void* dbias, int32_t dbias_dtype, int32_t dbias_accumulate, int32_t B, int32_t H, int32_t T,
                         int32_t head_dim, float scale, float p_drop, uint64_t seed, void* workspace, uint64_t ws_bytes,
                         void* stream);
int wl_colsum_finish(const float* part, int nblk, int n, void* out, int out_dtype, int accumulate, hipStream_t st);

struct WlFinSeg { const float* part; void* out; long stride, rep_stride; int nblk, n, out_dtype, accumulate, rep, blk0; };
#define WL_FIN_MAX 16
struct WlFinList { WlFinSeg s[WL_FIN_MAX]; int n, blocks; };
void wl_fin_defer(WlFinList* l);
bool wl_fin_active();
bool wl_fin_add(const float* part, int nblk, long stride, int n, void* out, int out_dtype, int accumulate, int rep = 1,
                long rep_stride = 0);
int wl_fin_flush(WlFinList& l, void* stream);
```

unispeech_amd/csrc/layer.hip:

```cpp
#include <stdlib.h>
#include <string.h>

#include <atomic>

#include "common.hpp"
#include "split_policy.hpp"
#include "wavlm_hip.h"

static std::atomic<wavlm_grad_listener> g_listener{nullptr};
static std::atomic<void*> g_listener_user{nullptr};
void wl_notify_grad(const void* base, uint64_t bytes, void* stream) {
  const wavlm_grad_listener cb = g_listener.load(std::memory_order_acquire);
  if (cb && base && bytes) cb(base, bytes, stream, g_listener_user.load(std::memory_order_acquire));
}
extern "C" void wavlm_dp_set_listener(wavlm_grad_listener cb, void* user) {
  g_listener.store(nullptr, std::memory_order_release);
  g_listener_user.store(user, std::memory_order_release);
  g_listener.store(cb, std::memory_order_release);
}

namespace {

inline uint64_t rup256(uint64_t v) { return (v + 255) & ~(uint64_t)255; }

// ... 187 lines not shown
      wavlm_gemm_desc g[4];
      for (int k = 0; k < m; ++k) {
        wg_desc(g[k], it[i + k], n, pdt, split);
        g[k].ws_bytes = wavlm_gemm_workspace_bytes(&g[k]);
        g[k].workspace = c.take(g[k].ws_bytes);
      }
      if (!c.ok) return WL_EINVAL;
      const int rc = wavlm_gemm_grouped(g, m, stream);
      if (rc != WL_OK) return rc;
    } else {
      wavlm_gemm_desc g;
      wg_desc(g, it[i], n, pdt, wavlm_split_single(it[i].N, it[i].K, kt, 0));
      if (g.split_k > 1) { g.ws_bytes = wavlm_gemm_workspace_bytes(&g); g.workspace = c.take(g.ws_bytes); if (!c.ok) return WL_EINVAL; }
      const int rc = wavlm_gemm(&g, stream);
      if (rc != WL_OK) return rc;
    }
    i = j;
  }
  return WL_OK;
}

uint64_t wavlm_layer_saved_bytes(const wavlm_layer_desc* d) { return desc_ok(d) ? carve_saved(d, nullptr).bytes : 0; }

uint64_t wavlm_layer_fwd_workspace_bytes(const wavlm_layer_desc* d) {
  if (!desc_ok(d)) return 0;
  return rup256((uint64_t)d->B * d->T * d->D * 2) + (d->saved ? 0 : carve_saved(d, nullptr).bytes);
}

uint64_t wavlm_layer_bwd_workspace_bytes(const wavlm_layer_desc* d) { return desc_ok(d) ? carve_bwd(d, nullptr, 0).bytes : 0; }

int wavlm_encoder_layer_fwd(const wavlm_layer_desc* d, void* stream) {
  if (!desc_ok(d) || !d->x || !d->y || !d->workspace) return WL_EINVAL;
  if (d->pre_ln && !d->r_out) return WL_EINVAL;
  if (d->ws_bytes < wavlm_layer_fwd_workspace_bytes(d)) return WL_EINVAL;
  const int64_t n = (int64_t)d->B * d->T;
  const int D = d->D, F = d->F, pdt = d->param_dtype;
  Carver wc(d->workspace, d->ws_bytes);
  void* tmp = wc.take((uint64_t)n * D * 2);
  void* sbase = d->saved;
  if (sbase) { if (d->saved_bytes < carve_saved(d, nullptr).bytes) return WL_EINVAL; }
  else sbase = wc.take(carve_saved(d, nullptr).bytes);
  if (!wc.ok) return WL_EINVAL;
  const Saved s = carve_saved(d, sbase);

  const void* ain = d->x;
  if (d->pre_ln) {
    RC(wavlm_layernorm_fwd(d->x, d->r_in, s.h1, d->r_in ? s.s1 : nullptr, s.mean1, s.rstd1, d->ln1_g, d->ln1_b, n, D, d->eps1,
                           WL_BF16, pdt, 0, d->r_in ? d->p_drop : 0.f, d->seed_r1, 0.f, 0, stream));
    ain = s.h1;
  }
  const float* gate = nullptr;
  if (d->Wgate) {
    RC(wavlm_gate_fwd(ain, d->Wgate, d->bgate, d->grep_a, s.gate, s.ga, s.gb, d->B, d->T, d->H, 64, WL_BF16, pdt, stream));
    gate = s.gate;
  } else if (d->tab) {
    return WL_EINVAL;
  }
  RC(lin_fwd(ain, d->Wqkv, d->bqkv, s.qkv, n, 3 * D, D, pdt, 0, nullptr, stream));
  RC(wavlm_attn_fused_fwd_p(s.qkv, s.O, s.lse, gate, d->tab, d->kpm, d->saved ? s.pstore : nullptr, s.pstore_b, d->B, d->H, d->T, 64,
                            d->scale, d->p_attn, d->seed_attn, stream));
  RC(lin_fwd(s.O, d->Wo, d->bo, tmp, n, D, D, pdt, 0, nullptr, stream));
  if (!d->pre_ln) {
    RC(wavlm_layernorm_fwd(d->x, tmp, s.x1, s.s1, s.mean1, s.rstd1, d->ln1_g, d->ln1_b, n, D, d->eps1, WL_BF16, pdt, 0,
                           d->p_drop, d->seed_r1, 0.f, 0, stream));
    RC(lin_fwd(s.x1, d->W1, d->b1, s.hact, n, F, D, pdt, 3, s.u, stream));
    RC(lin_fwd(s.hact, d->W2, d->b2, tmp, n, D, F, pdt, 0, nullptr, stream));
    RC(wavlm_layernorm_fwd(s.x1, tmp, d->y, s.s2, s.mean2, s.rstd2, d->ln2_g, d->ln2_b, n, D, d->eps2, WL_BF16, pdt, 0,
                           d->p_drop, d->seed_r2, 0.f, 0, stream));
  } else {
    const void* s1 = d->r_in ? s.s1 : d->x;
    RC(wavlm_layernorm_fwd(s1, tmp, s.x1, d->y, s.mean2, s.rstd2, d->ln2_g, d->ln2_b, n, D, d->eps2, WL_BF16, pdt, 0,
                           d->p_drop, d->seed_r2, 0.f, 0, stream));
    RC(lin_fwd(s.x1, d->W1, d->b1, s.hact, n, F, D, pdt, 3, s.u, stream));
    RC(lin_fwd(s.hact, d->W2, d->b2, d->r_out, n, D, F, pdt, 0, nullptr, stream));
  }
  return WL_OK;
}

int wavlm_encoder_layer_bwd(const wavlm_layer_desc* d, void* stream) {
  if (!desc_ok(d) || !d->x || !d->dy || !d->dx || !d->saved || !d->workspace) return WL_EINVAL;
  if (!d->dWqkv || !d->dbqkv || !d->dWo || !d->dbo || !d->dW1 || !d->db1 || !d->dW2 || (!d->db2 && !d->pre_ln)) return WL_EINVAL;
  if (!d->dln1_g || !d->dln1_b || !d->dln2_g || !d->dln2_b) return WL_EINVAL;
  if (d->Wgate && (!d->dWgate || !d->dbgate || !d->dgrep_a)) return WL_EINVAL;
  if (d->tab && (!d->dtab || !d->Wgate)) return WL_EINVAL;
  if (d->pre_ln && (!d->y || !d->dr_out || (d->r_in && !d->dr_in))) return WL_EINVAL;
  if (d->saved_bytes < carve_saved(d, nullptr).bytes) return WL_EINVAL;
  const int64_t n = (int64_t)d->B * d->T;
  const int D = d->D, F = d->F, pdt = d->param_dtype;
  const Saved s = carve_saved(d, d->saved);
  const BwdWs w = carve_bwd(d, d->workspace, d->ws_bytes);
  if (w.bytes == ~(uint64_t)0) return WL_EINVAL;
  const bool drop = d->p_drop > 0.f;
  WlFinList fin;
  struct Defer { Defer(WlFinList* l) { wl_fin_defer(l); } ~Defer() { wl_fin_defer(nullptr); } } defer(&fin);

  const void* df;
  const void* dres;
  if (!d->pre_ln) {
    RC(wavlm_layernorm_bwd(d->dy, s.s2, s.mean2, s.rstd2, d->ln2_g, d->ln2_b, w.dsa, drop ? w.df : nullptr, nullptr, d->dln2_g,
                           d->dln2_b, d->db2, n, D, WL_BF16, pdt, 0, d->p_drop, d->seed_r2, 0.f, 0, 1.f, 1, 0, w.ln_ws, w.ln_b, stream));
    df = drop ? w.df : w.dsa;
    dres = w.dsa;
  } else {
    df = d->dr_out;
    dres = nullptr;
    if (d->db2)
      RC(wavlm_colsum(df, n, D, D, WL_BF16, nullptr, nullptr, d->db2, pdt, 1, w.cs_ws2, w.cs_b, stream));
  }
  RC(lin_dx(df, d->W2, w.du, n, D, F, 4, s.u, nullptr, d->db1, pdt, w.cs_ws, w.cs_b, stream));
  RC(lin_dx(w.du, d->W1, w.dh, n, F, D, 0, nullptr, dres, nullptr, pdt, nullptr, 0, stream));

  const void* da;
  const void* dxres;
  if (!d->pre_ln) {
    RC(wavlm_layernorm_bwd(w.dh, s.s1, s.mean1, s.rstd1, d->ln1_g, d->ln1_b, w.dxa, drop ? w.da : nullptr, nullptr, d->dln1_g,
                           d->dln1_b, d->dbo, n, D, WL_BF16, pdt, 0, d->p_drop, d->seed_r1, 0.f, 0, 1.f, 1, 0, w.ln_ws2, w.ln_b, stream));
    da = drop ? w.da : w.dxa;
    dxres = w.dxa;
  } else {
    RC(wavlm_layernorm_bwd(w.dh, d->y, s.mean2, s.rstd2, d->ln2_g, d->ln2_b, w.dsa, drop ? w.da : nullptr, d->dy, d->dln2_g,
                           d->dln2_b, d->dbo, n, D, WL_BF16, pdt, 0, d->p_drop, d->seed_r2, 0.f, 0, 1.f, 1, 1, w.ln_ws, w.ln_b, stream));
    da = drop ? w.da : w.dsa;
    dxres = nullptr;
  }
  RC(lin_dx(da, d->Wo, w.dO, n, D, D, 0, nullptr, nullptr, nullptr, pdt, nullptr, 0, stream));
  RC(wl_attn_fused_bwd_ex(s.qkv, s.O, w.dO, s.lse, d->Wgate ? s.gate : nullptr, d->tab, d->kpm, s.pstore, s.pstore_b, w.dqkv, w.dgate, d->dtab,
                          d->dtab_accumulate, d->dbqkv, pdt, 1, d->B, d->H, d->T, 64, d->scale, d->p_attn, d->seed_attn, w.attn_ws,
                          w.attn_b, stream));
  const void* ain = d->pre_ln ? s.h1 : d->x;
  void* dain = d->pre_ln ? w.dxa : d->dx;
  RC(lin_dx(w.dqkv, d->Wqkv, dain, n, 3 * D, D, 0, nullptr, dxres, nullptr, pdt, nullptr, 0, stream));

  const wavlm_wgrad_item it[4] = {{df, s.hact, d->dW2, D, F}, {w.du, s.x1, d->dW1, F, D}, {da, s.O, d->dWo, D, D}, {w.dqkv, ain, d->dWqkv, 3 * D, D}};
  RC(wavlm_linear_wgrads(it, 4, n, pdt, w.wg_ws, w.wg_b, stream));

  if (d->Wgate)
    RC(wavlm_gate_bwd(w.dgate, ain, d->Wgate, d->grep_a, s.ga, s.gb, dain, d->dWgate, d->dbgate, d->dgrep_a, d->B, d->T, d->H, 64,
                      WL_BF16, pdt, 1 | 2, w.gate_ws, w.gate_b, stream));
  if (d->pre_ln) {
    const void* s1 = d->r_in ? s.s1 : d->x;
    RC(wavlm_layernorm_bwd(w.dxa, s1, s.mean1, s.rstd1, d->ln1_g, d->ln1_b, d->dx, (d->r_in && drop) ? d->dr_in : nullptr, w.dsa,
                           d->dln1_g, d->dln1_b, d->r_in ? d->db2_prev : nullptr, n, D, WL_BF16, pdt, 0, d->r_in ? d->p_drop : 0.f,
                           d->seed_r1, 0.f, 0, 1.f, 1, d->r_in ? 1 : 0, w.ln_ws2, w.ln_b, stream));
    if (d->r_in && !drop)
      RC(wavlm_axpby(d->dx, WL_BF16, d->dr_in, WL_BF16, n * D, 1.f, 0.f, stream));
  }
  wl_fin_defer(nullptr);
  return wl_fin_flush(fin, stream);
}

}
```

unispeech_amd/functional.py:

```python
import os
import threading
import weakref

import torch

from . import ops

_SEED_CTR = [0]
USE_FUSED_ATTENTION = True
_ASP = os.environ.get("WAVLM_ATTN_STORE_P", "0")
ATTN_STORE_P = True if _ASP == "1" else ("bits" if _ASP in ("bits", "2") else False)


def next_seed():
    _SEED_CTR[0] += 1
    return (torch.initial_seed() * 0x9E3779B97F4A7C15 + _SEED_CTR[0] * 0xD1B54A32D192ED03) & 0xFFFFFFFFFFFFFFFF


def _rup(x, m):
    return (x + m - 1) // m * m


CHAIN_CONSUMERS = os.environ.get("WAVLM_CHAIN_CONSUMERS", "1") == "1"
WGRAD_GROUPING = None
# ... 639 lines not shown
    def backward(ctx, dy):
        xg, u, Wb, norm, v, g = ctx.saved_tensors
        B, T, D, K, Cg, G, Tp = ctx.dims
        dyc = dy.contiguous()
        P = K - 1 - K // 2
        dug, du = ops.group_major(dyc, u, G, P, Tp, want_nat=True)
        dbias = ops.colsum(du.view(B * T, D), v.dtype)
        if ctx.direct and ops._lib.lib().wavlm_posconv_dw_direct_splits(Cg, G) > 0:
            dWf, nsplit = ops.posconv_dw_direct(xg, dug, P, T, K)
        else:
            dWfT = torch.empty((G, K * Cg, Cg), dtype=torch.float32, device=dy.device)
            ops.gemm(xg, dug, dWfT, K * Cg, Cg, T, lda=Cg, ldb=Cg, ldc=Cg, transA=True, transB=True,
                     b_off=P * Cg, KB=B, sA_kb=G * Tp * Cg, sB_kb=G * Tp * Cg, batch=(1, G),
                     sA=(0, Tp * Cg), sB=(0, Tp * Cg), sC=(0, Cg * K * Cg))
            dWf, nsplit = dWfT.transpose(1, 2).contiguous(), 1
        dv, dg = ops.posconv_weight_bwd(dWf, v.contiguous(), g.contiguous().view(-1), norm, nsplit=nsplit)
        dx = None
        if ctx.needs_input_grad[0]:
            dx = torch.empty_like(dyc)
            if ctx.direct:
                ops.posconv_direct(dug, Wb, dx, T, K, res=dyc)
            else:
                ops.gemm(dug, Wb, dx, T, Cg, K * Cg, lda=Cg, ldb=K * Cg, ldc=D, batch=(B, G),
                         sA=(G * Tp * Cg, Tp * Cg), sB=(0, Cg * K * Cg), sC=(T * D, Cg), res=dyc, ld_res=D,
                         sRes=(T * D, Cg))
        return dx, dv, dg.view_as(g), dbias, None


class RelPosTableFn(torch.autograd.Function):

    @staticmethod
    def forward(ctx, emb, bucket):
        H = emb.shape[1]
        tab = ops.relpos_gather(emb.contiguous(), bucket, H, bucket.numel())
        ctx.save_for_backward(emb, bucket)
        return tab

    @staticmethod
    def backward(ctx, dtab):
        emb, bucket = ctx.saved_tensors
        return ops.relpos_scatter(dtab.contiguous(), bucket, emb), None


class GateFn(torch.autograd.Function):

    @staticmethod
    def forward(ctx, x, W, bias, grep_a, H, pass_x=False):
        xc = x.contiguous()
        a = grep_a.contiguous().view(-1)
        gate, ga, gb = ops.gate_fwd(xc, W.contiguous(), bias.contiguous(), a, H)
        ctx.save_for_backward(xc, W, bias, grep_a, ga, gb)
        ctx.H = H
        if ctx.needs_input_grad[1]:
            for t in (W, bias, grep_a):
                _sink_use(t)
        return (gate, x.view_as(x)) if pass_x else gate

    @staticmethod
    def backward(ctx, dgate, dx_pass=None):
        xc, W, bias, grep_a, ga, gb = ctx.saved_tensors
        if dgate is None:
            return dx_pass, None, None, None, None, None
        sinks = (_sink(W), _sink(bias), _sink(grep_a))
        if any(t is None for t in sinks) or not (W.is_contiguous() and grep_a.is_contiguous()):
            sinks = None
        acc = None
        if dx_pass is not None and dx_pass.is_contiguous() and dx_pass.dtype == xc.dtype and ctx.needs_input_grad[0]:
            acc = dx_pass
        dx, dW, dbias, da = ops.gate_bwd(dgate.contiguous(), xc, W.contiguous(), bias, grep_a.contiguous().view(-1),
                                         ga, gb, ctx.H, sinks=None if sinks is None else tuple(t.view(-1) for t in sinks),
                                         dx_accumulate=acc)
        if acc is None and dx_pass is not None:
            dx = dx + dx_pass
        if sinks is not None:
            for t in sinks:
                _sink_written(t)
            return dx, None, None, None, None, None
        return dx, dW, dbias, da.view_as(grep_a), None, None


class AttnCoreFn(torch.autograd.Function):

    @staticmethod
    def forward(ctx, qkv, gate, tab, kpm, H, scale, p_drop, seed, qkv_bias_tok=None, qkv_bias_sink=None):
        B, T, D3 = qkv.shape
        D = D3 // 3
        hd = D // H
        dev = qkv.device
        qkvc = qkv.contiguous()
        ctx.fused = USE_FUSED_ATTENTION and qkv.dtype == torch.bfloat16 and hd == 64
        ctx.bias_sink = None
        if ctx.fused and qkv_bias_tok is not None and qkv_bias_sink is not None and ctx.needs_input_grad[0]:
            qkv_bias_tok.taken = True
            ctx.bias_sink = qkv_bias_sink
        if ctx.fused:
            store = ATTN_STORE_P if ctx.needs_input_grad[0] else False
            O, lse, pstore = ops.attn_fused_fwd(qkvc, gate, tab, kpm, H, scale, p_drop, seed, store_p=store)
            ctx.save_for_backward(qkvc, O, lse, gate, tab, kpm, pstore)
            ctx.cfg = (B, T, D, H, hd, 0, scale, p_drop, seed)
            return O
        ld = _rup(T, 8)
        S = torch.empty((B * H, T, ld), dtype=torch.float32, device=dev)
        ops.gemm(qkvc, qkvc, S, T, T, hd, lda=D3, ldb=D3, ldc=ld, batch=(B, H), sA=(T * D3, hd), sB=(T * D3, hd),
                 b_off=D, sC=(H * T * ld, T * ld), alpha=scale)
        P = torch.empty((B * H, T, ld), dtype=qkv.dtype, device=dev)
        lse = torch.empty((B * H, T), dtype=torch.float32, device=dev)
        ops.attn_softmax_fwd(S, P, lse, gate, tab, kpm, B, H, T, ld, ld, p_drop, seed)
        O = torch.empty((B, T, D), dtype=qkv.dtype, device=dev)
        ops.gemm(P, qkvc, O, T, hd, T, lda=ld, ldb=D3, ldc=D, transB=True, batch=(B, H), sA=(H * T * ld, T * ld),
                 sB=(T * D3, hd), b_off=2 * D, sC=(T * D, hd))
        ctx.save_for_backward(qkvc, S, P, lse, gate, tab, kpm)
        ctx.cfg = (B, T, D, H, hd, ld, scale, p_drop, seed)
        return O

    @staticmethod
    def backward(ctx, dO):
        if ctx.fused:
            qkvc, O, lse, gate, tab, kpm, pstore = ctx.saved_tensors
            B, T, D, H, hd, _, scale, p_drop, seed = ctx.cfg
            sb = ctx.bias_sink
            dqkv, dgate, dtab = ops.attn_fused_bwd(qkvc, O, dO.contiguous(), lse, gate, tab, kpm, H, scale, p_drop, seed,
                                                   dbias=sb.view(-1) if sb is not None else None, dbias_accumulate=True,
                                                   pstore=pstore)
            if sb is not None:
                _sink_written(sb)
            return dqkv, dgate, dtab, None, None, None, None, None, None, None
        qkvc, S, P, lse, gate, tab, kpm = ctx.saved_tensors
        B, T, D, H, hd, ld, scale, p_drop, seed = ctx.cfg
        D3 = 3 * D
        dev = dO.device
        dOc = dO.contiguous()
        dP = torch.empty((B * H, T, ld), dtype=P.dtype, device=dev)
        ops.gemm(dOc, qkvc, dP, T, T, hd, lda=D, ldb=D3, ldc=ld, batch=(B, H), sA=(T * D, hd), sB=(T * D3, hd),
                 b_off=2 * D, sC=(H * T * ld, T * ld))
        dS = torch.empty_like(dP)
        dgate = dtab = None
        if tab is not None:
            dgate = torch.empty((B, H, T), dtype=torch.float32, device=dev)
            dtab = torch.empty_like(tab)
        ops.attn_softmax_bwd(S, dP, lse, gate, tab, kpm, dS, dgate, dtab, B, H, T, ld, ld, p_drop, seed)
        dqkv = torch.empty_like(qkvc)
        ops.gemm(dS, qkvc, dqkv, T, hd, T, lda=ld, ldb=D3, ldc=D3, transB=True, batch=(B, H),
                 sA=(H * T * ld, T * ld), sB=(T * D3, hd), b_off=D, sC=(T * D3, hd), c_off=0, alpha=scale)
        ops.gemm(dS, qkvc, dqkv, T, hd, T, lda=ld, ldb=D3, ldc=D3, transA=True, transB=True, batch=(B, H),
                 sA=(H * T * ld, T * ld), sB=(T * D3, hd), b_off=0, sC=(T * D3, hd), c_off=D, alpha=scale)
        ops.gemm(P, dOc, dqkv, T, hd, T, lda=ld, ldb=D, ldc=D3, transA=True, transB=True, batch=(B, H),
                 sA=(H * T * ld, T * ld), sB=(T * D, hd), sC=(T * D3, hd), c_off=2 * D)
        return dqkv, dgate, dtab, None, None, None, None, None, None, None


class SelectRowsFn(torch.autograd.Function):

    @staticmethod
    def forward(ctx, x, sel, emb, zero):
        xc = x.contiguous()
        y = ops.select_rows(xc, sel, emb, zero)
        ctx.save_for_backward(sel, zero, emb)
        return y

    @staticmethod
    def backward(ctx, dy):
        sel, zero, emb = ctx.saved_tensors
        dyc = dy.contiguous()
        dx = ops.select_rows(dyc, sel, None, zero) if ctx.needs_input_grad[0] else None
        demb = None
        if emb is not None and sel is not None and ctx.needs_input_grad[2]:
            demb = ops.colsum(dyc.view(-1, dyc.shape[-1]), emb.dtype, include=sel, exclude=zero)
        return dx, None, demb, None


class GatherRowsFn(torch.autograd.Function):

    @staticmethod
    def forward(ctx, x2d, idx, inv_idx):
        ctx.save_for_backward(inv_idx)
        ctx.n = x2d.shape[0]
        if idx.numel() == 0:
            return x2d.new_empty((0, x2d.shape[1]))
        return ops.gather_rows(x2d.contiguous(), idx, idx.numel())

    @staticmethod
    def backward(ctx, dy):
        (inv_idx,) = ctx.saved_tensors
        if dy.shape[0] == 0:
            return dy.new_zeros((ctx.n, dy.shape[1])), None, None
        return ops.gather_rows(dy.contiguous(), inv_idx, ctx.n), None, None


class DropoutFn(torch.autograd.Function):
    @staticmethod
    def forward(ctx, x, p, seed):
        ctx.p, ctx.seed = p, seed
        return ops.dropout(x.contiguous(), p, seed)

    @staticmethod
    def backward(ctx, dy):
        return ops.dropout(dy.contiguous(), ctx.p, ctx.seed), None, None


def dropout(x, p, training=True):
    if not training or p <= 0:
        return x
    return DropoutFn.apply(x, p, next_seed())


class ReplaceMixFn(torch.autograd.Function):

    @staticmethod
    def forward(ctx, x, q, sel, p, seed):
        ctx.p, ctx.seed = p, seed
        ctx.save_for_backward(sel)
        return ops.replace_mix(x.contiguous(), q.contiguous(), sel, p, seed)

    @staticmethod
    def backward(ctx, dy):
        (sel,) = ctx.saved_tensors
        dx, dq = ops.replace_mix_bwd(dy.contiguous(), sel, ctx.p, ctx.seed)
        return dx, dq, None, None, None


def replace_mix(x, q, sel, p, training=True):
    live = training and p > 0
    return ReplaceMixFn.apply(x, q, sel, float(p) if live else 0.0, next_seed() if live else 0)


class MaskedPredLossFn(torch.autograd.Function):

    @staticmethod
    def forward(ctx, proj, label_embs, target, temp, need_grad):
        S, F = proj.shape
        V = label_embs.shape[0]
# ... 235 lines not shown
```

unispeech_amd/layerfn.py:

```python
import ctypes as C
import os
import weakref

import torch

from . import _lib, ops
from . import functional as F

LAYER_FUSED = os.environ.get("WAVLM_LAYER_FUSED", "1") != "0"


class TabGrad:
    __slots__ = ("buf",)

    def __init__(self):
        self.buf = None


def _ptr(t):
    return t.data_ptr() if t is not None else None


class _Binding:

    def __init__(self, layer):
        at = layer.self_attn
        pk = at._packed
        fc1, fc2 = layer.fc1, layer.fc2
        ln1, ln2 = layer.self_attn_layer_norm, layer.final_layer_norm
        d = _lib.LayerDesc()
        d.D, d.H, d.F = layer.embedding_dim, at.num_heads, fc1.weight.shape[0]
        d.pre_ln = int(bool(layer.layer_norm_first))
        d.param_dtype = ops.dt(fc1.weight)
        d.eps1, d.eps2, d.scale = ln1.eps, ln2.eps, at.scaling
        self.sinks = []

        def bind(name, p, explicit=None):
            g = explicit if explicit is not None else F._sink(p)
            if g is None:
                raise RuntimeError("parameter without a gradient sink")
            setattr(d, name, p.data_ptr())
            setattr(d, "d" + name, g.data_ptr())
            self.sinks.append((p if explicit is None else None, g))
            return g

        bind("Wqkv", pk[0], pk[1]); bind("bqkv", pk[2], pk[3])
        bind("Wo", at.out_proj.weight); bind("bo", at.out_proj.bias)
        bind("W1", fc1.weight); bind("b1", fc1.bias); bind("W2", fc2.weight)
        self.b2_sink = bind("b2", fc2.bias)
        self.b2_index = len(self.sinks) - 1
        bind("ln1_g", ln1.weight); bind("ln1_b", ln1.bias); bind("ln2_g", ln2.weight); bind("ln2_b", ln2.bias)
        self.gate_from = len(self.sinks)
        if at.gru_rel_pos:
            self.gate_ptrs = (at.grep_linear.weight.data_ptr(), at.grep_linear.bias.data_ptr(), at.grep_a.data_ptr())
            self.gate_sinks = tuple(F._sink(p) for p in (at.grep_linear.weight, at.grep_linear.bias, at.grep_a))
            if any(g is None for g in self.gate_sinks):
                raise RuntimeError("parameter without a gradient sink")
            self.gate_grad_ptrs = tuple(g.data_ptr() for g in self.gate_sinks)
        else:
            self.gate_ptrs = self.gate_sinks = self.gate_grad_ptrs = None
        self.desc = d
        self.key = (pk[0].data_ptr(), pk[1].data_ptr(), self.b2_sink.data_ptr(), fc2.weight.data_ptr())

    def valid_for(self, layer):
        pk = layer.self_attn._packed
        g = layer.fc2.bias.grad
        return (pk is not None and g is not None
                and self.key == (pk[0].data_ptr(), pk[1].data_ptr(), g.data_ptr(), layer.fc2.weight.data_ptr()))


_BINDINGS = weakref.WeakKeyDictionary()


def binding(layer):
    b = _BINDINGS.get(layer)
    if b is None or not b.valid_for(layer):
        b = _Binding(layer)
        _BINDINGS[layer] = b
    return b


def eligible(layer, x, table):
    if not (LAYER_FUSED and torch.is_grad_enabled() and x.is_cuda and x.dtype == torch.bfloat16 and x.dim() == 3):
        return False
    at = layer.self_attn
    if at.head_dim != 64 or layer.activation_name != "gelu" or not F.USE_FUSED_ATTENTION:
        return False
    if layer.training and layer.activation_dropout > 0:
        return False
    if (table is not None or at.has_relative_attention_bias) and not at.gru_rel_pos:
        return False
    pk = at._packed
    if pk is None or pk[0].dtype != x.dtype or pk[0].data_ptr() != at.q_proj.weight.data_ptr() or pk[2].data_ptr() != at.q_proj.bias.data_ptr():
        return False
    ps = [at.out_proj.weight, at.out_proj.bias, layer.fc1.weight, layer.fc1.bias, layer.fc2.weight, layer.fc2.bias,
          layer.self_attn_layer_norm.weight, layer.self_attn_layer_norm.bias, layer.final_layer_norm.weight,
          layer.final_layer_norm.bias]
    if at.gru_rel_pos:
        ps += [at.grep_linear.weight, at.grep_linear.bias, at.grep_a]
# ... 7 lines not shown

    @staticmethod
    def forward(ctx, x, r_in, tab, layer, kpm, tabgrad, owns_tab, prev_tok, out_tok):
        bd = binding(layer)
        B, T, D = x.shape
        xc = x if x.is_contiguous() else x.contiguous()
        rc = None
        if r_in is not None:
            rc = r_in if r_in.is_contiguous() else r_in.contiguous()
        training = layer.training
        p_drop = layer.dropout if training else 0.0
        p_attn = layer.self_attn.dropout_module.p if training else 0.0
        d = _lib.LayerDesc()
        C.memmove(C.byref(d), C.byref(bd.desc), C.sizeof(d))
        d.B, d.T = B, T
        d.p_drop, d.p_attn = p_drop, p_attn
        d.attn_store_p = 2 if F.ATTN_STORE_P == "bits" else int(bool(F.ATTN_STORE_P))
        if d.pre_ln and p_drop > 0 and rc is not None:
            d.seed_r1 = F.next_seed()
        if p_attn > 0:
            d.seed_attn = F.next_seed()
        if not d.pre_ln and p_drop > 0:
            d.seed_r1 = F.next_seed()
        if p_drop > 0:
            d.seed_r2 = F.next_seed()
        use_tab = tab is not None
        if use_tab:
            d.tab = tab.data_ptr()
            d.Wgate, d.bgate, d.grep_a = bd.gate_ptrs
        d.kpm = _ptr(kpm)
        d.x, d.r_in = xc.data_ptr(), _ptr(rc)
        y = torch.empty_like(xc)
        d.y = y.data_ptr()
        r_out = None
        if d.pre_ln:
            r_out = torch.empty_like(xc)
            d.r_out = r_out.data_ptr()
        L = _lib.lib()
        nsaved = int(L.wavlm_layer_saved_bytes(C.byref(d)))
        saved = torch.empty(nsaved, dtype=torch.uint8, device=x.device)
        d.saved, d.saved_bytes = saved.data_ptr(), nsaved
        need = int(L.wavlm_layer_fwd_workspace_bytes(C.byref(d)))
        ws = ops.workspace(x.device, need, "layer")
        d.workspace, d.ws_bytes = ws.data_ptr(), need
        _lib.check(L.wavlm_encoder_layer_fwd(C.byref(d), ops.stream()), "wavlm_encoder_layer_fwd")
        ctx.desc, ctx.bd, ctx.use_tab, ctx.tabgrad, ctx.owns_tab = d, bd, use_tab, tabgrad, owns_tab
        ctx.prev_sink = None
        if prev_tok is not None and rc is not None:
            ps = F._sink(prev_tok.param)
            if ps is not None:
                prev_tok.taken = True
                ctx.prev_sink = ps
        ctx.out_tok = out_tok
        if F.SINK_LISTENERS:
            for p, g in bd.sinks:
                F._sink_use(p, g)
            if use_tab:
                for g in bd.gate_sinks:
                    F._sink_use(None, g)
        ctx.save_for_backward(xc, rc, y if d.pre_ln else None, saved, tab, kpm)
        if d.pre_ln:
            return y, r_out
        return y

    @staticmethod
    def backward(ctx, dy, dr_out=None):
        xc, rc, y, saved, tab, kpm = ctx.saved_tensors
        d, bd = ctx.desc, ctx.bd
        dev = xc.device
        if d.pre_ln:
            if dy is None or dr_out is None:
                raise NotImplementedError("fused pre-LN block: both outputs must be used")
            dr_out = dr_out if dr_out.is_contiguous() else dr_out.contiguous()
            d.dr_out = dr_out.data_ptr()
            d.y = y.data_ptr()
        dy = dy if dy.is_contiguous() else dy.contiguous()
        d.dy = dy.data_ptr()
        dx = torch.empty_like(xc)
        d.dx = dx.data_ptr()
        dr_in = None
        if rc is not None:
            dr_in = torch.empty_like(xc)
            d.dr_in = dr_in.data_ptr()
        tg = ctx.tabgrad
        if ctx.use_tab:
            d.dWgate, d.dbgate, d.dgrep_a = bd.gate_grad_ptrs
            if tg.buf is None:
                tg.buf = torch.empty_like(tab)
                d.dtab_accumulate = 0
            else:
                d.dtab_accumulate = 1
            d.dtab = tg.buf.data_ptr()
        b2_here = True
        if d.pre_ln:
            b2_here = not (ctx.out_tok is not None and ctx.out_tok.taken)
            if not b2_here:
                d.db2 = None
            d.db2_prev = _ptr(ctx.prev_sink)
        L = _lib.lib()
        need = int(L.wavlm_layer_bwd_workspace_bytes(C.byref(d)))
        ws = ops.workspace(dev, need, "layer")
        d.workspace, d.ws_bytes = ws.data_ptr(), need
        _lib.check(L.wavlm_encoder_layer_bwd(C.byref(d), ops.stream()), "wavlm_encoder_layer_bwd")
        if F.SINK_LISTENERS:
            for i, (_p, g) in enumerate(bd.sinks):
                if i == bd.b2_index and not b2_here:
                    continue
                F._sink_written(g)
            if ctx.use_tab:
                for g in bd.gate_sinks:
                    F._sink_written(g)
            if ctx.prev_sink is not None:
                F._sink_written(ctx.prev_sink)
        dtab = tg.buf if (ctx.use_tab and ctx.owns_tab) else None
        return dx, dr_in, dtab, None, None, None, None, None, None


def run_block(layer, x, kpm, table, r_in=None, prev_tok=None, out_tok=None):
    at = layer.self_attn
    if at.has_relative_attention_bias and table is None:
        table = at.position_table(x.shape[1], x.device)
    tab_in, tg, owns = None, None, False
    if table is not None:
        tg = getattr(table, "_wl_tabgrad", None)
        if tg is None:
            tg = table._wl_tabgrad = TabGrad()
            owns = True
        tab_in = table if owns else table.detach()
    out = EncoderLayerFn.apply(x, r_in, tab_in, layer, kpm, tg, owns, prev_tok, out_tok)
    if layer.layer_norm_first:
        return out[0], out[1], table
    return out, None, table
```

unispeech_amd/ops.py:

```python
import ctypes as C
import math
import os

import torch

from . import _lib
from ._lib import BF16, F32, ConvRelayoutDesc, GemmDesc, check

_WS = {}


def dt(t):
    if t.dtype == torch.float32:
        return F32
    if t.dtype == torch.bfloat16:
        return BF16
    raise TypeError("unsupported dtype %s (float32 / bfloat16 only)" % t.dtype)


def _dev(t):
    if not t.is_cuda:
        raise _lib.WavlmHipError("unispeech_amd kernels need a HIP device tensor (no CPU fallback)")
    return t.device

# ... 444 lines not shown
    return tab


def relpos_scatter(dtab, bucket, like_emb):
    H, L_ = dtab.shape
    demb = torch.empty_like(like_emb)
    check(_lib.lib().wavlm_relpos_scatter(ptr(dtab), ptr(bucket), ptr(demb), dt(demb), H, L_, like_emb.shape[0],
                                          stream()), "wavlm_relpos_scatter")
    return demb


def gate_fwd(x, W, bias, grep_a, H):
    dev = _dev(x); _contig(x)
    B, T, D = x.shape
    hd = D // H
    gate = torch.empty((B, H, T), dtype=torch.float32, device=dev)
    ga = torch.empty_like(gate)
    gb = torch.empty_like(gate)
    check(_lib.lib().wavlm_gate_fwd(ptr(x), ptr(W), ptr(bias), ptr(grep_a), ptr(gate), ptr(ga), ptr(gb), B, T, H, hd,
                                    dt(x), dt(W), stream()), "wavlm_gate_fwd")
    return gate, ga, gb


def gate_bwd(dgate, x, W, bias, grep_a, ga, gb, H, sinks=None, dx_accumulate=None):
    dev = _dev(x)
    B, T, D = x.shape
    hd = D // H
    dx = dx_accumulate if dx_accumulate is not None else torch.empty_like(x)
    _contig(dx)
    if sinks is not None:
        dW, dbias, da = sinks
    else:
        dW = torch.empty_like(W)
        dbias = torch.empty_like(bias)
        da = torch.empty_like(grep_a)
    L = _lib.lib()
    need = L.wavlm_gate_bwd_workspace_bytes(H, hd)
    ws = workspace(dev, need)
    check(L.wavlm_gate_bwd(ptr(dgate), ptr(x), ptr(W), ptr(grep_a), ptr(ga), ptr(gb), ptr(dx), ptr(dW), ptr(dbias),
                           ptr(da), B, T, H, hd, dt(x), dt(W), int(sinks is not None) | (2 if dx_accumulate is not None else 0),
                           ptr(ws), need, stream()),
          "wavlm_gate_bwd")
    if sinks is not None:
        return dx, None, None, None
    return dx, dW, dbias, da


def attn_softmax_fwd(S, P, lse, gate, tab, kpm, B, H, T, ldS, ldP, p_drop, seed):
    check(_lib.lib().wavlm_attn_softmax_fwd(ptr(S), ptr(P), ptr(lse), ptr(gate), ptr(tab), ptr(kpm), B, H, T, ldS, ldP,
                                            dt(S), dt(P), float(p_drop), int(seed), stream()),
          "wavlm_attn_softmax_fwd")


def attn_softmax_bwd(S, dP, lse, gate, tab, kpm, dS, dgate, dtab, B, H, T, ldS, ldP, p_drop, seed):
    dev = _dev(S)
    L = _lib.lib()
    need = L.wavlm_attn_softmax_bwd_workspace_bytes(B, H, T) if tab is not None else 0
    ws = workspace(dev, need) if need else None
    check(L.wavlm_attn_softmax_bwd(ptr(S), ptr(dP), ptr(lse), ptr(gate), ptr(tab), ptr(kpm), ptr(dS), ptr(dgate),
                                   ptr(dtab), 0, B, H, T, ldS, ldP, dt(S), dt(dS), float(p_drop), int(seed), ptr(ws),
                                   need, stream()), "wavlm_attn_softmax_bwd")


def attn_fused_fwd(qkv, gate, tab, kpm, H, scale, p_drop, seed, store_p=False):
    dev = _dev(qkv); _contig(qkv)
    B, T, D3 = qkv.shape
    D = D3 // 3
    O = torch.empty((B, T, D), dtype=qkv.dtype, device=dev)
    lse = torch.empty((B * H, T), dtype=torch.float32, device=dev)
    L = _lib.lib()
    pstore, nps = None, 0
    if store_p == "bits":
        if p_drop > 0:
            nps = int(L.wavlm_attn_fused_dbits_bytes(B, H, T))
            pstore = torch.empty(nps, dtype=torch.uint8, device=dev)
    elif store_p:
        nps = int(L.wavlm_attn_fused_pstore_bytes(B, H, T))
        pstore = torch.empty(nps, dtype=torch.uint8, device=dev) if nps else None
    check(L.wavlm_attn_fused_fwd_p(ptr(qkv), ptr(O), ptr(lse), ptr(gate), ptr(tab), ptr(kpm), ptr(pstore), nps, B, H, T, D // H,
                                   float(scale), float(p_drop), int(seed), stream()), "wavlm_attn_fused_fwd_p")
    return O, lse, pstore


def attn_fused_bwd(qkv, O, dO, lse, gate, tab, kpm, H, scale, p_drop, seed, dbias=None, dbias_accumulate=False, pstore=None):
    dev = _dev(qkv); _contig(dO)
    B, T, D3 = qkv.shape
    D = D3 // 3
    dqkv = torch.empty_like(qkv)
    dgate = dtab = None
    if tab is not None:
        dgate = torch.empty((B, H, T), dtype=torch.float32, device=dev)
        dtab = torch.empty_like(tab)
    L = _lib.lib()
    need = L.wavlm_attn_fused_bwd_workspace_bytes(B, H, T)
    ws = workspace(dev, need, "attn")
    check(L.wavlm_attn_fused_bwd_p(ptr(qkv), ptr(O), ptr(dO), ptr(lse), ptr(gate), ptr(tab), ptr(kpm), ptr(pstore),
                                   pstore.numel() if pstore is not None else 0, ptr(dqkv),
                                   ptr(dgate), ptr(dtab), ptr(dbias), dt(dbias) if dbias is not None else 0,
                                   int(bool(dbias_accumulate)), B, H, T, D // H, float(scale), float(p_drop), int(seed),
                                   ptr(ws), need, stream()), "wavlm_attn_fused_bwd_p")
    return dqkv, dgate, dtab


def posconv_weight_fwd(v, g, out_dtype, layout=0):
    dev = _dev(v); _contig(v)
    D, Cg, K = v.shape
    G = D // Cg
    Wf = torch.empty((G, Cg, K * Cg), dtype=out_dtype, device=dev)
    Wb = torch.empty((G, Cg, K * Cg), dtype=out_dtype, device=dev)
    norm = torch.empty(K, dtype=torch.float32, device=dev)
    L = _lib.lib()
    need = L.wavlm_posconv_weight_workspace_bytes(D, Cg, K)
    ws = workspace(dev, need)
    check(L.wavlm_posconv_weight_fwd(ptr(v), ptr(g), dt(v), ptr(Wf), ptr(Wb), dt(Wf), ptr(norm), D, Cg, K, int(layout),
                                     ptr(ws), need, stream()), "wavlm_posconv_weight_fwd")
    return Wf, Wb, norm


def posconv_weight_bwd(dWf, v, g, norm, nsplit=1):
    dev = _dev(v)
    D, Cg, K = v.shape
    dv = torch.empty_like(v)
    dg = torch.empty_like(g)
    L = _lib.lib()
    need = L.wavlm_posconv_weight_workspace_bytes(D, Cg, K)
    ws = workspace(dev, need)
    check(L.wavlm_posconv_weight_bwd(ptr(dWf), ptr(v), ptr(g), ptr(norm), dt(v), ptr(dv), ptr(dg), D, Cg, K, int(nsplit),
                                     ptr(ws), need, stream()), "wavlm_posconv_weight_bwd")
    return dv, dg


def group_major(x, aux, G, left_pad, Tp, want_nat=False, aux_is_grad=False):
    dev = _dev(x); _contig(x); _contig(aux)
    B, T, D = x.shape
    out = torch.empty((B, G, Tp, D // G), dtype=x.dtype, device=dev)
    nat = torch.empty_like(x) if want_nat else None
    check(_lib.lib().wavlm_posconv_group_major(ptr(x), ptr(aux), ptr(out), ptr(nat), B, T, D, G, left_pad, Tp, dt(x),
                                               int(bool(aux_is_grad)), stream()), "wavlm_posconv_group_major")
    return out, nat


def posconv_dw_direct(xg, dug, du_off, T, K):
    dev = _dev(xg); _contig(xg); _contig(dug)
    B, G, Tp, Cg = xg.shape
    L = _lib.lib()
    S = L.wavlm_posconv_dw_direct_splits(Cg, G)
    if S <= 0:
        raise ValueError("posconv_dw_direct: shape not covered")
    part = torch.empty((S, G, Cg, K * Cg), dtype=torch.float32, device=dev)
    check(L.wavlm_posconv_dw_direct(ptr(xg), ptr(dug), ptr(part), B, G, T, Tp, int(du_off), Cg, K, stream()),
          "wavlm_posconv_dw_direct")
    return part, S


def posconv_direct_supported(x_dtype, Cg, K, T):
    return x_dtype == torch.bfloat16 and bool(_lib.lib().wavlm_posconv_direct_supported(int(Cg), int(K), int(T)))


def posconv_direct(xg, W, out, T, K, *, bias=None, res=None, aux=None, gelu=False):
    _dev(xg); _contig(xg); _contig(W); _contig(out); _contig(res); _contig(aux)
    B, G, Tp, Cg = xg.shape
    check(_lib.lib().wavlm_posconv_direct(ptr(xg), ptr(W), ptr(bias), ptr(res), ptr(out), ptr(aux), B, G, T, Tp, Cg, K,
                                          int(bool(gelu)), stream()), "wavlm_posconv_direct")
    return out


def l2norm_fwd(x, out_dtype, eps=1e-8):
    dev = _dev(x); _contig(x)
    rows, D = x.shape
    y = torch.empty((rows, D), dtype=out_dtype, device=dev)
    inv = torch.empty(rows, dtype=torch.float32, device=dev)
    check(_lib.lib().wavlm_l2norm_fwd(ptr(x), dt(x), ptr(y), dt(y), ptr(inv), rows, D, float(eps), stream()),
          "wavlm_l2norm_fwd")
    return y, inv


def l2norm_bwd(dy, y, inv, x_dtype):
    dev = _dev(dy); _contig(dy)
    rows, D = y.shape
    dx = torch.empty((rows, D), dtype=x_dtype, device=dev)
    check(_lib.lib().wavlm_l2norm_bwd(ptr(dy), ptr(y), dt(y), ptr(inv), ptr(dx), dt(dx), rows, D, stream()),
          "wavlm_l2norm_bwd")
    return dx
# ... 443 lines not shown
```

unispeech_amd/wavlm.py:

```python
import math
import os
from typing import List, Optional, Tuple

import numpy as np
import torch
import torch.nn as nn

from . import functional as F
from . import layerfn
from .masking import compute_mask_indices, relative_position_buckets


class WavLMConfig:

    def __init__(self, cfg=None):
        self.extractor_mode: str = "default"
        self.encoder_layers: int = 12
        self.encoder_embed_dim: int = 768
        self.encoder_ffn_embed_dim: int = 3072
        self.encoder_attention_heads: int = 12
        self.activation_fn: str = "gelu"
        self.layer_norm_first: bool = False
        self.conv_feature_layers: str = "[(512,10,5)] + [(512,3,2)] * 4 + [(512,2,2)] * 2"
        self.conv_bias: bool = False
# ... 139 lines not shown
    def _tag_pack_owner(self):
        for lin in (self.q_proj, self.k_proj, self.v_proj):
            lin.weight._wl_pack_owner = self
            lin.bias._wl_pack_owner = self

    def __setstate__(self, state):
        super().__setstate__(state)
        self.__dict__.pop("_packed_w", None)
        self.__dict__.pop("_packed_b", None)
        self.__dict__.pop("_wl_binding", None)
        self._packed = None
        self._tag_pack_owner()

    def _apply(self, fn, recurse=True):
        out = super()._apply(fn, recurse)
        self._tag_pack_owner()
        return out

    def reset_parameters(self):
        g = 1 / math.sqrt(2)
        nn.init.xavier_uniform_(self.k_proj.weight, gain=g)
        nn.init.xavier_uniform_(self.v_proj.weight, gain=g)
        nn.init.xavier_uniform_(self.q_proj.weight, gain=g)
        nn.init.xavier_uniform_(self.out_proj.weight)
        nn.init.constant_(self.out_proj.bias, 0.0)
        if self.has_relative_attention_bias:
            nn.init.xavier_normal_(self.relative_attention_bias.weight)

    def packed_param_groups(self):
        D = self.embed_dim

        def bind_w(pv, gv):
            self._packed_w = (pv.view(3 * D, D), gv.view(3 * D, D))
            self._refresh_packed()

        def bind_b(pv, gv):
            self._packed_b = (pv.view(3 * D), gv.view(3 * D))
            self._refresh_packed()

        return [([self.q_proj.weight, self.k_proj.weight, self.v_proj.weight], bind_w),
                ([self.q_proj.bias, self.k_proj.bias, self.v_proj.bias], bind_b)]

    def _refresh_packed(self):
        w, b = getattr(self, "_packed_w", None), getattr(self, "_packed_b", None)
        self._packed = (w[0], w[1], b[0], b[1]) if (w is not None and b is not None) else None

    def position_table(self, T, device):
        key = (int(T), str(device))
        cache = self.__dict__.setdefault("_bucket_cache", {})
        bucket = cache.get(key)
        if bucket is None:
            if len(cache) > 64:
                cache.clear()
            bucket = relative_position_buckets(T, self.num_buckets, self.max_distance).to(device)
            cache[key] = bucket
        return F.RelPosTableFn.apply(self.relative_attention_bias.weight, bucket)

    def forward(self, x, key_padding_u8=None, position_table=None, out_bias_tok=None, wgroup=None, chain=False):
        B, T, D = x.shape
        if self.has_relative_attention_bias and position_table is None:
            position_table = self.position_table(T, x.device)
        gate = None
        if position_table is not None:
            if self.gru_rel_pos:
                if chain:
                    gate, x = F.GateFn.apply(x, self.grep_linear.weight, self.grep_linear.bias, self.grep_a, self.num_heads, True)
                else:
                    gate = F.GateFn.apply(x, self.grep_linear.weight, self.grep_linear.bias, self.grep_a, self.num_heads)
            else:
                gate = torch.ones((B, self.num_heads, T), dtype=torch.float32, device=x.device)
        pk = self._packed
        if (pk is not None and torch.is_grad_enabled() and pk[0].data_ptr() == self.q_proj.weight.data_ptr()
                and pk[2].data_ptr() == self.q_proj.bias.data_ptr() and pk[0].dtype == x.dtype):
            tq = F.BiasGradToken(pk[2])
            qkv = F.LinearFn.apply(x, pk[0], pk[2], pk[1], pk[3], tq, wgroup, chain)
        else:
            tq = None
            srcs = [self.q_proj.weight, self.k_proj.weight, self.v_proj.weight, self.q_proj.bias, self.k_proj.bias, self.v_proj.bias]
            w, b = F.eval_derived(srcs, "qkv_packed", lambda: (torch.cat(srcs[:3], dim=0), torch.cat(srcs[3:], dim=0)))
            qkv = F.LinearFn.apply(x, w, b, None, None, None, None, chain)
        if chain:
            qkv, x = qkv
        p = self.dropout_module.p if self.training else 0.0
        o = F.AttnCoreFn.apply(qkv, gate, position_table, key_padding_u8, self.num_heads, self.scaling, p,
                               F.next_seed() if p > 0 else 0, tq, pk[3] if tq is not None else None)
        out = F.LinearFn.apply(o, self.out_proj.weight, self.out_proj.bias, None, None, out_bias_tok, wgroup)
        return (out, position_table, x) if chain else (out, position_table)


PRELN_FUSED = os.environ.get("WAVLM_PRELN_FUSED", "1") != "0"


class ResidualAddFn(torch.autograd.Function):

    @staticmethod
    def forward(ctx, x, r, p, seed):
        from . import ops
        xc, rc = x.contiguous(), r.contiguous()
        if xc.numel() % 8 == 0:
            y = ops.dropout_add(xc, rc, p, seed)
        else:
            y = xc.clone()
            ops.axpby_(y, ops.dropout(rc, p, seed) if p > 0 else rc, 1.0, 1.0)
        ctx.p, ctx.seed = p, seed
        return y

    @staticmethod
    def backward(ctx, dy):
        from . import ops
        dr = ops.dropout(dy.contiguous(), ctx.p, ctx.seed) if ctx.p > 0 else dy
        return dy, dr, None, None


ACTIVATION_FNS = ("relu", "gelu", "gelu_accurate", "tanh", "linear", "glu")


class GLULinear(nn.Module):

    def __init__(self, input_dim, output_dim):
        super().__init__()
        self.output_dim = output_dim
        self.linear = nn.Linear(input_dim, output_dim * 2)


class TransformerSentenceEncoderLayer(nn.Module):

    def __init__(self, embedding_dim=768, ffn_embedding_dim=3072, num_attention_heads=8, dropout=0.1,
                 attention_dropout=0.1, activation_dropout=0.1, activation_fn="relu", layer_norm_first=False,
                 has_relative_attention_bias=False, num_buckets=0, max_distance=0, gru_rel_pos=False):
        super().__init__()
        if activation_fn == "gelu_fast":
            activation_fn = "gelu_accurate"
        if activation_fn not in ACTIVATION_FNS:
            raise RuntimeError("--activation-fn {} not supported".format(activation_fn))
        self.activation_name = activation_fn
        self.embedding_dim = embedding_dim
        self.dropout = dropout
        self.activation_dropout = activation_dropout
        self.self_attn = MultiheadAttention(embedding_dim, num_attention_heads, dropout=attention_dropout,
                                            has_relative_attention_bias=has_relative_attention_bias,
                                            num_buckets=num_buckets, max_distance=max_distance, gru_rel_pos=gru_rel_pos)
        self.dropout1 = nn.Dropout(dropout)
        self.dropout2 = nn.Dropout(activation_dropout)
        self.dropout3 = nn.Dropout(dropout)
        self.layer_norm_first = layer_norm_first
        self.self_attn_layer_norm = nn.LayerNorm(embedding_dim)
        if activation_fn == "glu":
            self.fc1 = GLULinear(embedding_dim, ffn_embedding_dim)
        else:
            self.fc1 = nn.Linear(embedding_dim, ffn_embedding_dim)
        self.fc2 = nn.Linear(ffn_embedding_dim, embedding_dim)
        self.final_layer_norm = nn.LayerNorm(embedding_dim)

    def _ffn(self, x, b2_tok=None, wgroup=None, chain=False):
        p = self.activation_dropout if self.training else 0.0
        fc1 = self.fc1.linear if self.activation_name == "glu" else self.fc1
        return F.infer_apply(F.FFNFn, x, fc1.weight, fc1.bias, self.fc2.weight, self.fc2.bias, p,
                             F.next_seed() if p > 0 else 0, b2_tok, wgroup, chain, self.activation_name)

    def forward_preln_fused(self, x, pending, key_padding_u8=None, position_table=None):
        ln1, ln2 = self.self_attn_layer_norm, self.final_layer_norm
        p = self.dropout if self.training else 0.0
        if layerfn.eligible(self, x, position_table):
            tf = F.BiasGradToken(self.fc2.bias)
            x, f, position_table = layerfn.run_block(self, x, key_padding_u8, position_table,
                                                     r_in=None if pending is None else pending[0],
                                                     prev_tok=None if pending is None else pending[1], out_tok=tf)
            return x, (f, tf), position_table
# ... 304 lines not shown
```

Measured before the change: 15370 audio-s/s.

## Accumulate shared relative-position table gradient in partials across layers, reduce once

Instead of each layer's attention backward running a separate dtab reduction kernel and handing a full table gradient to autograd, the shared position table gradient now accumulates into a per-(batch, head, q-tile) partial buffer that every non-owning layer adds into, with the kernel reading the old value during its skewed-sum flush. Only the owning (first-created, last-backward) layer runs the final reduce kernel. This removes eleven reduce launches and the autograd-side table gradient additions, at the cost of an extra read per partial write in the kernel and a persistent partial buffer whose size grows with B*H*T.

```diff
diff --git a/include/wavlm_hip.h b/include/wavlm_hip.h
--- a/include/wavlm_hip.h
+++ b/include/wavlm_hip.h
@@ -160,6 +160,15 @@
                            float* dgate, float* dtab, void* dbias, int32_t dbias_dtype, int32_t dbias_accumulate, int32_t B,
                            int32_t H, int32_t T, int32_t head_dim, float scale, float p_drop, uint64_t seed, void* workspace,
                            uint64_t ws_bytes, void* stream);
+#define WAVLM_DTAB_PART_ADD 1
+#define WAVLM_DTAB_DEFER 2
+uint64_t wavlm_attn_fused_dtab_part_bytes(int32_t B, int32_t H, int32_t T);
+int wavlm_attn_fused_bwd_shared(const void* qkv, const void* O, const void* dO, const float* lse, const float* gate,
+                                const float* tab, const uint8_t* kpm, const void* pstore, uint64_t pstore_bytes, void* dqkv,
+                                float* dgate, float* dtab, int32_t dtab_accumulate, float* dtab_part, int32_t dtab_flags,
+                                void* dbias, int32_t dbias_dtype, int32_t dbias_accumulate, int32_t B, int32_t H, int32_t T,
+                                int32_t head_dim, float scale, float p_drop, uint64_t seed, void* workspace, uint64_t ws_bytes,
+                                void* stream);
 
 uint64_t wavlm_posconv_weight_workspace_bytes(int32_t D, int32_t Cg, int32_t K);
 int wavlm_posconv_weight_fwd(const void* v, const void* g, int32_t param_dtype, void* Wf, void* Wb, int32_t out_dtype,
@@ -226,6 +235,7 @@
   float eps1, eps2, scale;
   float p_drop, p_attn;
   int32_t attn_store_p;
+  int32_t dtab_flags;
   uint64_t seed_r1, seed_r2, seed_attn;
   const void *Wqkv, *bqkv, *Wo, *bo, *W1, *b1, *W2, *b2, *ln1_g, *ln1_b, *ln2_g, *ln2_b;
   const void *Wgate, *bgate, *grep_a;
@@ -244,6 +254,7 @@
   void* dx;
   void* dr_in;
   float* dtab;
+  float* dtab_part;
 } wavlm_layer_desc;
 uint64_t wavlm_layer_saved_bytes(const wavlm_layer_desc* d);
 uint64_t wavlm_layer_fwd_workspace_bytes(const wavlm_layer_desc* d);
diff --git a/unispeech_amd/_lib.py b/unispeech_amd/_lib.py
--- a/unispeech_amd/_lib.py
+++ b/unispeech_amd/_lib.py
@@ -47,7 +47,7 @@
         ("B", c_i32), ("T", c_i32), ("D", c_i32), ("H", c_i32), ("F", c_i32),
         ("pre_ln", c_i32), ("param_dtype", c_i32), ("dtab_accumulate", c_i32),
         ("eps1", c_f32), ("eps2", c_f32), ("scale", c_f32), ("p_drop", c_f32), ("p_attn", c_f32),
-        ("attn_store_p", c_i32),
+        ("attn_store_p", c_i32), ("dtab_flags", c_i32),
         ("seed_r1", c_u64), ("seed_r2", c_u64), ("seed_attn", c_u64),
         ("Wqkv", c_vp), ("bqkv", c_vp), ("Wo", c_vp), ("bo", c_vp), ("W1", c_vp), ("b1", c_vp), ("W2", c_vp), ("b2", c_vp),
         ("ln1_g", c_vp), ("ln1_b", c_vp), ("ln2_g", c_vp), ("ln2_b", c_vp),
@@ -59,9 +59,11 @@
         ("tab", c_vp), ("kpm", c_vp),
         ("x", c_vp), ("r_in", c_vp), ("y", c_vp), ("r_out", c_vp),
         ("saved", c_vp), ("saved_bytes", c_u64), ("workspace", c_vp), ("ws_bytes", c_u64),
-        ("dy", c_vp), ("dr_out", c_vp), ("dx", c_vp), ("dr_in", c_vp), ("dtab", c_vp),
+        ("dy", c_vp), ("dr_out", c_vp), ("dx", c_vp), ("dr_in", c_vp), ("dtab", c_vp), ("dtab_part", c_vp),
     ]
 
+
+DTAB_PART_ADD, DTAB_DEFER = 1, 2
 
 GRAD_LISTENER = C.CFUNCTYPE(None, c_vp, c_u64, c_vp, c_vp)
 
@@ -135,6 +137,10 @@
                                        c_u64, c_vp]),
     "wavlm_attn_fused_bwd_p": (c_i32, [c_vp, c_vp, c_vp, c_vp, c_vp, c_vp, c_vp, c_vp, c_u64, c_vp, c_vp, c_vp, c_vp, c_i32, c_i32,
                                        c_i32, c_i32, c_i32, c_i32, c_f32, c_f32, c_u64, c_vp, c_u64, c_vp]),
+    "wavlm_attn_fused_dtab_part_bytes": (c_u64, [c_i32, c_i32, c_i32]),
+    "wavlm_attn_fused_bwd_shared": (c_i32, [c_vp, c_vp, c_vp, c_vp, c_vp, c_vp, c_vp, c_vp, c_u64, c_vp, c_vp, c_vp, c_i32, c_vp,
+                                            c_i32, c_vp, c_i32, c_i32, c_i32, c_i32, c_i32, c_i32, c_f32, c_f32, c_u64, c_vp,
+                                            c_u64, c_vp]),
     "wavlm_posconv_weight_workspace_bytes": (c_u64, [c_i32, c_i32, c_i32]),
     "wavlm_posconv_weight_fwd": (c_i32, [c_vp, c_vp, c_i32, c_vp, c_vp, c_i32, c_vp, c_i32, c_i32, c_i32, c_i32, c_vp,
                                          c_u64, c_vp]),
diff --git a/unispeech_amd/csrc/attn_fused.hip b/unispeech_amd/csrc/attn_fused.hip
--- a/unispeech_amd/csrc/attn_fused.hip
+++ b/unispeech_amd/csrc/attn_fused.hip
@@ -511,6 +511,8 @@
 
   float pend_v = 0.f;
   int pend_d = -1;
+  float pend_old = 0.f;
+  const bool dadd = TAB && p.dtab_add;
   auto skew_sums = [&](int j0p) __attribute__((always_inline)) {
     f32x4_t nacc[6];
 #pragma unroll
@@ -540,8 +542,19 @@
     pend_d = dlo0 + j0p + lane;
   };
   auto flush_pending = [&]() __attribute__((always_inline)) {
-    if (pend_d >= 0 && pend_d < L) prow[pend_d] = pend_v;
+#if FA_DQ_DEFER
+    if (dadd && pend_d >= 0 && pend_d < L) pend_old = prow[pend_d];
+#endif
+    if (pend_d >= 0 && pend_d < L) prow[pend_d] = pend_v + pend_old;
     pend_d = -1;
+  };
+  auto fetch_old = [&](int j0n) __attribute__((always_inline)) {
+#if !FA_DQ_DEFER
+    if (dadd) {
+      const int dn = dlo0 + j0n + lane;
+      if (dn >= 0 && dn < L) pend_old = prow[dn];
+    }
+#endif
   };
   int cur = 0;
   auto tile_body = [&](int jt, U4 (&x0)[2], U4 (&x1)[2], float& mx) __attribute__((always_inline)) {
@@ -563,7 +576,7 @@
       FA_LOAD_KV(j0 + FA_BKV, kbuf(cur ^ 1), vbuf(cur ^ 1));
     }
     if constexpr (SP && !(FA_SP_PROBE & 1)) p_load(jt + 2 < nkv ? jt + 2 : jt, x0, x1, mx);
-    if constexpr (TAB) flush_pending();
+    if constexpr (TAB) { flush_pending(); fetch_old(j0); }
     unsigned bw0 = 0, bw1 = 0;
     if constexpr (BCONS) {
       bw0 = nxt0 >> (8 * (1 - hi)); bw1 = nxt1 >> (8 * (1 - hi));
@@ -791,7 +804,7 @@
   if (TAB && lane < 32) {
     const float v = lane < 16 ? dacc[4][0] : dacc[5][0];
     const int d = dlo0 + 64 * nkv + lane;
-    if (d >= 0 && d < L) prow[d] = v;
+    if (d >= 0 && d < L) prow[d] = dadd ? v + prow[d] : v;
   }
 #if FA_DQ_PK
   dg = dg2[0] + dg2[1];
@@ -890,6 +903,7 @@
   p.Ltab = (T + p.Tkb + 3) & ~3;
   p.qkv = nullptr; p.O = nullptr; p.lse = nullptr; p.gate = nullptr; p.tab = nullptr; p.kpm = nullptr;
   p.dO = nullptr; p.dqkv = nullptr; p.delta = nullptr; p.dgate = nullptr; p.dtab_part = nullptr; p.dbias_part = nullptr;
+  p.dtab_add = 0;
   return p;
 }
 
@@ -957,7 +971,7 @@
                          const float* tab, const uint8_t* kpm, void* dqkv, float* dgate, float* dtab, void* dbias,
                          int32_t dbias_dtype, int32_t dbias_accumulate, int32_t B, int32_t H, int32_t T, int32_t head_dim,
                          float scale, float p_drop, uint64_t seed, void* workspace, uint64_t ws_bytes, void* stream) {
-  return wl_attn_fused_bwd_ex(qkv, O, dO, lse, gate, tab, kpm, nullptr, 0, dqkv, dgate, dtab, 0, dbias, dbias_dtype, dbias_accumulate,
+  return wl_attn_fused_bwd_ex(qkv, O, dO, lse, gate, tab, kpm, nullptr, 0, dqkv, dgate, dtab, 0, nullptr, 0, dbias, dbias_dtype, dbias_accumulate,
                               B, H, T, head_dim, scale, p_drop, seed, workspace, ws_bytes, stream);
 }
 
@@ -968,22 +982,43 @@
                            uint64_t ws_bytes, void* stream) {
   if (pstore && pstore_bytes == fa_dbits_bytes(B, H, T)) { if ((uintptr_t)pstore & 255) return WL_EINVAL; }
   else if (pstore && (T > FA_PSTORE_MAX_T || pstore_bytes < wavlm_attn_fused_pstore_bytes(B, H, T) || ((uintptr_t)pstore & 15))) return WL_EINVAL;
-  return wl_attn_fused_bwd_ex(qkv, O, dO, lse, gate, tab, kpm, pstore, pstore_bytes, dqkv, dgate, dtab, 0, dbias, dbias_dtype, dbias_accumulate,
+  return wl_attn_fused_bwd_ex(qkv, O, dO, lse, gate, tab, kpm, pstore, pstore_bytes, dqkv, dgate, dtab, 0, nullptr, 0, dbias, dbias_dtype, dbias_accumulate,
                               B, H, T, head_dim, scale, p_drop, seed, workspace, ws_bytes, stream);
+}
+
+uint64_t wavlm_attn_fused_dtab_part_bytes(int32_t B, int32_t H, int32_t T) {
+  if (B <= 0 || H <= 0 || T <= 0) return 0;
+  const uint64_t nqt = (uint64_t)((T + FA_BQ - 1) / FA_BQ), Lp = (2 * (uint64_t)T - 1 + 3) & ~(uint64_t)3;
+  return (uint64_t)B * H * nqt * 4 * Lp * sizeof(float);
+}
+
+int wavlm_attn_fused_bwd_shared(const void* qkv, const void* O, const void* dO, const float* lse, const float* gate,
+                                const float* tab, const uint8_t* kpm, const void* pstore, uint64_t pstore_bytes, void* dqkv,
+                                float* dgate, float* dtab, int32_t dtab_accumulate, float* dtab_part, int32_t dtab_flags,
+                                void* dbias, int32_t dbias_dtype, int32_t dbias_accumulate, int32_t B, int32_t H, int32_t T,
+                                int32_t head_dim, float scale, float p_drop, uint64_t seed, void* workspace, uint64_t ws_bytes,
+                                void* stream) {
+  if (pstore && pstore_bytes == fa_dbits_bytes(B, H, T)) { if ((uintptr_t)pstore & 255) return WL_EINVAL; }
+  else if (pstore && (T > FA_PSTORE_MAX_T || pstore_bytes < wavlm_attn_fused_pstore_bytes(B, H, T) || ((uintptr_t)pstore & 15))) return WL_EINVAL;
+  return wl_attn_fused_bwd_ex(qkv, O, dO, lse, gate, tab, kpm, pstore, pstore_bytes, dqkv, dgate, dtab, dtab_accumulate, dtab_part, dtab_flags,
+                              dbias, dbias_dtype, dbias_accumulate, B, H, T, head_dim, scale, p_drop, seed, workspace, ws_bytes, stream);
 }
 
 }
 
 int wl_attn_fused_bwd_ex(const void* qkv, const void* O, const void* dO, const float* lse, const float* gate,
                          const float* tab, const uint8_t* kpm, const void* pstore, uint64_t pstore_bytes, void* dqkv, float* dgate,
-                         float* dtab, int dtab_accumulate,
+                         float* dtab, int dtab_accumulate, float* dtab_part, int dtab_flags,
                          void* dbias, int32_t dbias_dtype, int32_t dbias_accumulate, int32_t B, int32_t H, int32_t T,
                          int32_t head_dim, float scale, float p_drop, uint64_t seed, void* workspace, uint64_t ws_bytes,
                          void* stream) {
   if (!qkv || !O || !dO || !lse || !dqkv || !workspace || B <= 0 || H <= 0 || T <= 0 || head_dim != FA_HD)
     return WL_EINVAL;
   if ((gate == nullptr) != (tab == nullptr)) return WL_EINVAL;
-  if (tab && (!dgate || !dtab)) return WL_EINVAL;
+  const bool dtab_defer = tab && (dtab_flags & WAVLM_DTAB_DEFER);
+  if (tab && (!dgate || (!dtab && !dtab_defer))) return WL_EINVAL;
+  if ((dtab_flags & ~(WAVLM_DTAB_PART_ADD | WAVLM_DTAB_DEFER)) || (dtab_flags && !dtab_part)) return WL_EINVAL;
+  if (dtab_part && ((uintptr_t)dtab_part & 15)) return WL_EINVAL;
   if (ws_bytes < wavlm_attn_fused_bwd_workspace_bytes(B, H, T)) return WL_EINVAL;
   hipStream_t st = (hipStream_t)stream;
   FaP p = fa_params(B, H, T, scale, p_drop, seed);
@@ -994,9 +1029,10 @@
   if (pstore) fa_bind_pstore(p, const_cast<void*>(pstore), B, H, T);
   const int nqt = (T + FA_BQ - 1) / FA_BQ;
   const int L = 2 * T - 1;
-  p.dtab_part = (float*)workspace;
   const int Lp = (L + 3) & ~3;
-  p.delta = p.dtab_part + (long)B * H * nqt * 4 * Lp;
+  p.delta = (float*)workspace + (long)B * H * nqt * 4 * Lp;
+  p.dtab_part = dtab_part ? dtab_part : (float*)workspace;
+  p.dtab_add = (tab && (dtab_flags & WAVLM_DTAB_PART_ADD)) ? 1 : 0;
   if (dbias) p.dbias_part = p.delta + (long)B * H * T;
   static const bool dbits_on = []() { const char* e = getenv("WAVLM_ATTN_DBITS"); return e && e[0] == '1'; }();
   static const bool dkv64_on = []() { const char* e = getenv("WAVLM_ATTN_DKV64"); return e && e[0] == '1'; }();
@@ -1055,7 +1091,7 @@
     if (rcb != WL_OK) return rcb;
     if (dbias_accumulate && !wl_fin_active()) wl_notify_grad(dbias, (uint64_t)3 * H * FA_HD * wl_esize(dbias_dtype), stream);
   }
-  if (tab)
+  if (tab && !dtab_defer)
     WL_LAUNCH(fa_dtab_reduce_kernel, dim3((unsigned)((Lp / 4 + 15) / 16), (unsigned)H), dim3(1024), 0, st,
               (const float*)p.dtab_part, dtab, (int)B, (int)H, nqt, L, Lp, (int)T, (T + FA_BKV - 1) / FA_BKV, (int)dtab_accumulate);
   return wl_check_launch();
diff --git a/unispeech_amd/csrc/attn_fused.hpp b/unispeech_amd/csrc/attn_fused.hpp
--- a/unispeech_amd/csrc/attn_fused.hpp
+++ b/unispeech_amd/csrc/attn_fused.hpp
@@ -129,6 +129,7 @@
   FaPstore ps;
   unsigned* dbits; int db_nkb, db_Tq;
   int db_fwd;
+  int dtab_add;
   int Ltab, Tkb;
   int nqb;
 };
diff --git a/unispeech_amd/csrc/common.hpp b/unispeech_amd/csrc/common.hpp
--- a/unispeech_amd/csrc/common.hpp
+++ b/unispeech_amd/csrc/common.hpp
@@ -188,7 +188,7 @@
 static inline uint64_t wl_esize(int dt) { return dt == WL_BF16 ? 2 : 4; }
 int wl_attn_fused_bwd_ex(const void* qkv, const void* O, const void* dO, const float* lse, const float* gate,
                          const float* tab, const uint8_t* kpm, const void* pstore, uint64_t pstore_bytes, void* dqkv, float* dgate,
-                         float* dtab, int dtab_accumulate,
+                         float* dtab, int dtab_accumulate, float* dtab_part, int dtab_flags,
                          void* dbias, int32_t dbias_dtype, int32_t dbias_accumulate, int32_t B, int32_t H, int32_t T,
                          int32_t head_dim, float scale, float p_drop, uint64_t seed, void* workspace, uint64_t ws_bytes,
                          void* stream);
diff --git a/unispeech_amd/csrc/layer.hip b/unispeech_amd/csrc/layer.hip
--- a/unispeech_amd/csrc/layer.hip
+++ b/unispeech_amd/csrc/layer.hip
@@ -293,7 +293,7 @@
   if (!d->dWqkv || !d->dbqkv || !d->dWo || !d->dbo || !d->dW1 || !d->db1 || !d->dW2 || (!d->db2 && !d->pre_ln)) return WL_EINVAL;
   if (!d->dln1_g || !d->dln1_b || !d->dln2_g || !d->dln2_b) return WL_EINVAL;
   if (d->Wgate && (!d->dWgate || !d->dbgate || !d->dgrep_a)) return WL_EINVAL;
-  if (d->tab && (!d->dtab || !d->Wgate)) return WL_EINVAL;
+  if (d->tab && ((!d->dtab && !(d->dtab_flags & WAVLM_DTAB_DEFER)) || !d->Wgate)) return WL_EINVAL;
   if (d->pre_ln && (!d->y || !d->dr_out || (d->r_in && !d->dr_in))) return WL_EINVAL;
   if (d->saved_bytes < carve_saved(d, nullptr).bytes) return WL_EINVAL;
   const int64_t n = (int64_t)d->B * d->T;
@@ -336,7 +336,7 @@
   }
   RC(lin_dx(da, d->Wo, w.dO, n, D, D, 0, nullptr, nullptr, nullptr, pdt, nullptr, 0, stream));
   RC(wl_attn_fused_bwd_ex(s.qkv, s.O, w.dO, s.lse, d->Wgate ? s.gate : nullptr, d->tab, d->kpm, s.pstore, s.pstore_b, w.dqkv, w.dgate, d->dtab,
-                          d->dtab_accumulate, d->dbqkv, pdt, 1, d->B, d->H, d->T, 64, d->scale, d->p_attn, d->seed_attn, w.attn_ws,
+                          d->dtab_accumulate, d->dtab_part, d->dtab_flags, d->dbqkv, pdt, 1, d->B, d->H, d->T, 64, d->scale, d->p_attn, d->seed_attn, w.attn_ws,
                           w.attn_b, stream));
   const void* ain = d->pre_ln ? s.h1 : d->x;
   void* dain = d->pre_ln ? w.dxa : d->dx;
diff --git a/unispeech_amd/functional.py b/unispeech_amd/functional.py
--- a/unispeech_amd/functional.py
+++ b/unispeech_amd/functional.py
@@ -745,7 +745,8 @@
 class AttnCoreFn(torch.autograd.Function):
 
     @staticmethod
-    def forward(ctx, qkv, gate, tab, kpm, H, scale, p_drop, seed, qkv_bias_tok=None, qkv_bias_sink=None):
+    def forward(ctx, qkv, gate, tab, kpm, H, scale, p_drop, seed, qkv_bias_tok=None, qkv_bias_sink=None, tabgrad=None,
+                owns_tab=True):
         B, T, D3 = qkv.shape
         D = D3 // 3
         hd = D // H
@@ -753,6 +754,7 @@
         qkvc = qkv.contiguous()
         ctx.fused = USE_FUSED_ATTENTION and qkv.dtype == torch.bfloat16 and hd == 64
         ctx.bias_sink = None
+        ctx.tabgrad, ctx.owns_tab = (tabgrad, owns_tab) if (ctx.fused and tab is not None) else (None, True)
         if ctx.fused and qkv_bias_tok is not None and qkv_bias_sink is not None and ctx.needs_input_grad[0]:
             qkv_bias_tok.taken = True
             ctx.bias_sink = qkv_bias_sink
@@ -784,10 +786,10 @@
             sb = ctx.bias_sink
             dqkv, dgate, dtab = ops.attn_fused_bwd(qkvc, O, dO.contiguous(), lse, gate, tab, kpm, H, scale, p_drop, seed,
                                                    dbias=sb.view(-1) if sb is not None else None, dbias_accumulate=True,
-                                                   pstore=pstore)
+                                                   pstore=pstore, tabgrad=ctx.tabgrad, owns_tab=ctx.owns_tab)
             if sb is not None:
                 _sink_written(sb)
-            return dqkv, dgate, dtab, None, None, None, None, None, None, None
+            return dqkv, dgate, dtab, None, None, None, None, None, None, None, None, None
         qkvc, S, P, lse, gate, tab, kpm = ctx.saved_tensors
         B, T, D, H, hd, ld, scale, p_drop, seed = ctx.cfg
         D3 = 3 * D
@@ -809,7 +811,7 @@
                  sA=(H * T * ld, T * ld), sB=(T * D3, hd), b_off=0, sC=(T * D3, hd), c_off=D, alpha=scale)
         ops.gemm(P, dOc, dqkv, T, hd, T, lda=ld, ldb=D, ldc=D3, transA=True, transB=True, batch=(B, H),
                  sA=(H * T * ld, T * ld), sB=(T * D, hd), sC=(T * D3, hd), c_off=2 * D)
-        return dqkv, dgate, dtab, None, None, None, None, None, None, None
+        return dqkv, dgate, dtab, None, None, None, None, None, None, None, None, None
 
 
 class SelectRowsFn(torch.autograd.Function):
diff --git a/unispeech_amd/layerfn.py b/unispeech_amd/layerfn.py
--- a/unispeech_amd/layerfn.py
+++ b/unispeech_amd/layerfn.py
@@ -11,10 +11,29 @@
 
 
 class TabGrad:
-    __slots__ = ("buf",)
+    __slots__ = ("part",)
 
     def __init__(self):
-        self.buf = None
+        self.part = None
+
+    def enter(self, lib, tab, B, H, T, owns):
+        flags = 0 if owns else _lib.DTAB_DEFER
+        part = self.part
+        if part is None:
+            n = int(lib.wavlm_attn_fused_dtab_part_bytes(B, H, T))
+            part = torch.empty(n // 4, dtype=torch.float32, device=tab.device)
+        else:
+            flags |= _lib.DTAB_PART_ADD
+        self.part = None if owns else part
+        return part, (torch.empty_like(tab) if owns else None), flags
+
+
+def share_table(table):
+    tg = getattr(table, "_wl_tabgrad", None)
+    owns = tg is None
+    if owns:
+        tg = table._wl_tabgrad = TabGrad()
+    return (table if owns else table.detach()), tg, owns
 
 
 def _ptr(t):
@@ -188,22 +207,19 @@
         if rc is not None:
             dr_in = torch.empty_like(xc)
             d.dr_in = dr_in.data_ptr()
-        tg = ctx.tabgrad
+        dtab = None
+        L = _lib.lib()
         if ctx.use_tab:
             d.dWgate, d.dbgate, d.dgrep_a = bd.gate_grad_ptrs
-            if tg.buf is None:
-                tg.buf = torch.empty_like(tab)
-                d.dtab_accumulate = 0
-            else:
-                d.dtab_accumulate = 1
-            d.dtab = tg.buf.data_ptr()
+            part, dtab, d.dtab_flags = ctx.tabgrad.enter(L, tab, d.B, d.H, d.T, ctx.owns_tab)
+            d.dtab_accumulate = 0
+            d.dtab_part, d.dtab = part.data_ptr(), _ptr(dtab)
         b2_here = True
         if d.pre_ln:
             b2_here = not (ctx.out_tok is not None and ctx.out_tok.taken)
             if not b2_here:
                 d.db2 = None
             d.db2_prev = _ptr(ctx.prev_sink)
-        L = _lib.lib()
         need = int(L.wavlm_layer_bwd_workspace_bytes(C.byref(d)))
         ws = ops.workspace(dev, need, "layer")
         d.workspace, d.ws_bytes = ws.data_ptr(), need
@@ -218,7 +234,6 @@
                     F._sink_written(g)
             if ctx.prev_sink is not None:
                 F._sink_written(ctx.prev_sink)
-        dtab = tg.buf if (ctx.use_tab and ctx.owns_tab) else None
         return dx, dr_in, dtab, None, None, None, None, None, None
 
 
@@ -228,11 +243,7 @@
         table = at.position_table(x.shape[1], x.device)
     tab_in, tg, owns = None, None, False
     if table is not None:
-        tg = getattr(table, "_wl_tabgrad", None)
-        if tg is None:
-            tg = table._wl_tabgrad = TabGrad()
-            owns = True
-        tab_in = table if owns else table.detach()
+        tab_in, tg, owns = share_table(table)
     out = EncoderLayerFn.apply(x, r_in, tab_in, layer, kpm, tg, owns, prev_tok, out_tok)
     if layer.layer_norm_first:
         return out[0], out[1], table
diff --git a/unispeech_amd/ops.py b/unispeech_amd/ops.py
--- a/unispeech_amd/ops.py
+++ b/unispeech_amd/ops.py
@@ -550,23 +550,29 @@
     return O, lse, pstore
 
 
-def attn_fused_bwd(qkv, O, dO, lse, gate, tab, kpm, H, scale, p_drop, seed, dbias=None, dbias_accumulate=False, pstore=None):
+def attn_fused_bwd(qkv, O, dO, lse, gate, tab, kpm, H, scale, p_drop, seed, dbias=None, dbias_accumulate=False, pstore=None,
+                   tabgrad=None, owns_tab=True):
     dev = _dev(qkv); _contig(dO)
     B, T, D3 = qkv.shape
     D = D3 // 3
     dqkv = torch.empty_like(qkv)
-    dgate = dtab = None
+    dgate = dtab = part = None
+    flags = 0
+    L = _lib.lib()
     if tab is not None:
         dgate = torch.empty((B, H, T), dtype=torch.float32, device=dev)
-        dtab = torch.empty_like(tab)
-    L = _lib.lib()
+        if tabgrad is not None:
+            part, dtab, flags = tabgrad.enter(L, tab, B, H, T, owns_tab)
+        else:
+            dtab = torch.empty_like(tab)
     need = L.wavlm_attn_fused_bwd_workspace_bytes(B, H, T)
     ws = workspace(dev, need, "attn")
-    check(L.wavlm_attn_fused_bwd_p(ptr(qkv), ptr(O), ptr(dO), ptr(lse), ptr(gate), ptr(tab), ptr(kpm), ptr(pstore),
-                                   pstore.numel() if pstore is not None else 0, ptr(dqkv),
-                                   ptr(dgate), ptr(dtab), ptr(dbias), dt(dbias) if dbias is not None else 0,
-                                   int(bool(dbias_accumulate)), B, H, T, D // H, float(scale), float(p_drop), int(seed),
-                                   ptr(ws), need, stream()), "wavlm_attn_fused_bwd_p")
+    check(L.wavlm_attn_fused_bwd_shared(ptr(qkv), ptr(O), ptr(dO), ptr(lse), ptr(gate), ptr(tab), ptr(kpm), ptr(pstore),
+                                        pstore.numel() if pstore is not None else 0, ptr(dqkv),
+                                        ptr(dgate), ptr(dtab), 0, ptr(part), flags, ptr(dbias),
+                                        dt(dbias) if dbias is not None else 0,
+                                        int(bool(dbias_accumulate)), B, H, T, D // H, float(scale), float(p_drop), int(seed),
+                                        ptr(ws), need, stream()), "wavlm_attn_fused_bwd_shared")
     return dqkv, dgate, dtab
 
 
diff --git a/unispeech_amd/wavlm.py b/unispeech_amd/wavlm.py
--- a/unispeech_amd/wavlm.py
+++ b/unispeech_amd/wavlm.py
@@ -245,8 +245,12 @@
         if chain:
             qkv, x = qkv
         p = self.dropout_module.p if self.training else 0.0
-        o = F.AttnCoreFn.apply(qkv, gate, position_table, key_padding_u8, self.num_heads, self.scaling, p,
-                               F.next_seed() if p > 0 else 0, tq, pk[3] if tq is not None else None)
+        tab_in, tg, owns = position_table, None, True
+        if (position_table is not None and torch.is_grad_enabled() and F.USE_FUSED_ATTENTION and qkv.dtype == torch.bfloat16
+                and self.head_dim == 64):
+            tab_in, tg, owns = layerfn.share_table(position_table)
+        o = F.AttnCoreFn.apply(qkv, gate, tab_in, key_padding_u8, self.num_heads, self.scaling, p,
+                               F.next_seed() if p > 0 else 0, tq, pk[3] if tq is not None else None, tg, owns)
         out = F.LinearFn.apply(o, self.out_proj.weight, self.out_proj.bias, None, None, out_bias_tok, wgroup)
         return (out, position_table, x) if chain else (out, position_table)
 
```

Result: no change. 15410 audio-s/s (median of 6 runs) (+0.3%).
